# larq/compute-engine

Hardware: AMD Instinct MI355X
Metric: binary-MACs/sec (LceBconv2d 3x3 256->256, 56x56, batch 256/GPU, f32 out) (higher is better)
Workload: dtype fp4-e2m1 (exact +-1) matrix-core dot product, fp32 accumulate, f32 epilogue

## Files before the change

compute-engine_amd/csrc/lce_dispatch_stream.h:

```cpp
#pragma once
#include "../../include/lce_hip.h"
#include "lce_kernel_types.h"
#include "lce_kernels_stream.h"

namespace lce {

template <int DST, bool FAST, bool CLAMP, bool SIGN, bool I8F>
stream_fn stream_by_kch(int kch, bool strips) {
  if (strips)
    return kch == 4 ? bconv2d_stream<DST, 3, 3, 4, FAST, CLAMP, SIGN, false, true, I8F> : nullptr;
  switch (kch) {
    case 8: return bconv2d_stream<DST, 3, 3, 8, FAST, CLAMP, SIGN, true, false, I8F>;
    case 4: return bconv2d_stream<DST, 3, 3, 4, FAST, CLAMP, SIGN, false, false, I8F>;
    case 2: return bconv2d_stream<DST, 3, 3, 2, FAST, CLAMP, SIGN, false, false, I8F>;
    case 1: return bconv2d_stream<DST, 3, 3, 1, FAST, CLAMP, SIGN, false, false, I8F>;
    default: return nullptr;
  }
}
template <int DST, bool CLAMP, bool SIGN, bool I8F = false>
stream_fn stream_by_fast(int kch, bool fast, bool strips) {
  return fast ? stream_by_kch<DST, true, CLAMP, SIGN, I8F>(kch, strips) : stream_by_kch<DST, false, CLAMP, SIGN, I8F>(kch, strips);
}
template <int DST, bool CLAMP, bool I8F>
stream_fn find_stream_part(int kch, bool fast, bool sign, bool strips) {
  if constexpr (DST == kDstBitpacked) return stream_by_fast<kDstBitpacked, false, false>(kch, fast, strips);
  else return sign ? stream_by_fast<DST, CLAMP, true, I8F>(kch, fast, strips) : stream_by_fast<DST, CLAMP, false, I8F>(kch, fast, strips);
}

}
```

compute-engine_amd/csrc/lce_kernel_args.h:

```cpp
#pragma once
#include <stdint.h>
#include "lce_experiments.h"

namespace lce {

enum : int { kDstFloat = 0, kDstInt8 = 1, kDstBitpacked = 2 };

enum : int {
  kZeroPadNone = 0,
  kZeroPadExact = 1,
  kZeroPadCorrection = 2,
};

struct FastDiv {
  uint32_t magic;
  uint32_t shift;
};

inline FastDiv make_fastdiv(uint32_t d) {
  FastDiv f{0u, 0u};
  if (d <= 1) return f;
  uint32_t l = 0;
  while ((1ull << l) < d) ++l;
  const uint64_t two = 1ull << (31 + l);
  f.magic = (uint32_t)((two + d - 1) / d);
  f.shift = l - 1;
  return f;
}
struct FastDivNB {
  uint32_t magic;
  uint32_t shift;
  uint32_t pass;
};
inline FastDivNB make_fastdiv_nb(uint32_t d) {
  const FastDiv f = make_fastdiv(d);
  return FastDivNB{f.magic, f.shift, f.magic == 0u ? 0xffffffffu : 0u};
}

struct ConvArgs {
  int32_t H, W;
  int32_t Cw, Cwg;
  int32_t OH, OW;
  int32_t N, Npg;
  int32_t KH, KW, SH, SW, DH, DW, PH, PW;
  int32_t M;
  int32_t PT, NT;
  int32_t Wout;
  uint32_t in_bytes;
  FastDiv div_ow, div_oh;
  int32_t clamp_min, clamp_max;
  int32_t zero_pad_mode;
  int32_t bzp;
  int32_t eKH, eKW;
  int32_t left_off, top_off;
};


struct MfmaArgs {
  int32_t H, W, Cw, Cin;
  int32_t Hp, Wp, PH, PW;
  uint32_t NPIX;
  int32_t CPW;
  int32_t KCH;
  int32_t Npad;
  int32_t zero_border;
  uint32_t x_bytes, w_bytes;
  FastDiv div_npix, div_wp, div_hp;
  float a_bt;
  float cmin, cmax;
  int32_t TPI;
  int32_t OHOW;
  int32_t halo_rows;
  int32_t PS;
  int32_t halo_bytes;
  int32_t QG;
  int32_t IPT;
  int32_t B;
  int32_t HPIX;
  int32_t f32_wide;
  int32_t i8_wide;
  int32_t noclamp;
  float bit_thr;
  FastDiv div_tpi, div_qg, div_ohow, div_hpix;
  FastDiv div_npg;
  int32_t Wh, TX;
  FastDiv div_wh, div_tx;
};


struct PwArgs {
  int32_t M;
  int32_t N;
  int32_t Npad;
  int32_t Cw;
  int32_t Cin;
  int32_t Wout;
  int32_t tiles;
  int32_t noclamp;
  uint32_t in_bytes;
  uint32_t out_bytes;
  float a_bt;
  float cmin, cmax;
  float bit_thr;
  int32_t OW, OHW;
  int32_t IW, IHW;
  int32_t SH, SW;
  FastDiv div_ow, div_ohw;
};



constexpr int kStreamItemsPerLane = 2;
struct StreamArgs {
  int32_t H, W, Cw, Cin;
  int32_t OH, OW, N, Npad, Wout;
  int32_t SH, SW, PH, PW;
  int32_t B;
  int32_t Wp;
  int32_t pitch;
  int32_t R;
  int32_t ring_bytes;
  int32_t zero_border;
  int32_t QG;
  int32_t IPR;
  int32_t RS;
  int32_t SPI;
  int32_t SRS;
  int32_t PBS;
  int32_t S;
  int32_t SPB;
  int32_t GSTR, G0M, GX;
  int32_t pph_log;
  int32_t NSTRIP, RSEG, WSo, XS0;
  int32_t flat;
  int32_t NPX;
  int32_t NQ;
  uint32_t need0;
  uint32_t in_bytes, w_bytes, out_bytes;
  uint32_t tab_bytes, tab_lim, tab_ctx, tab_sgn;
  uint32_t tab_seg;
  uint32_t sign_bytes;
  float a_bt, cmin, cmax, bit_thr;
  FastDivNB div_ipr, div_qg, div_srs, div_spi, div_r, div_rseg, div_gstr;
};


struct WsArgs {
  int32_t H, W, Cw, Cin;
  int32_t OH, OW, N, Npad, Wout;
  int32_t SH, SW, PH, PW;
  int32_t B;
  int32_t IPB;
  int32_t GROUPS;
  int32_t PARTS;
  int32_t NPXG;
  int32_t NQ;
  int32_t Hp, Wp;
  int32_t pitch, img_pitch;
  int32_t QG;
  int32_t items;
  int32_t zero_border;
  int32_t noclamp;
  uint32_t lds_images;
  uint32_t in_bytes, w_bytes, out_bytes, sign_bytes, tab_bytes;
  uint32_t tab_part, tab_ctx;
  float a_bt, cmin, cmax, bit_thr;
  FastDivNB div_qg, div_wp, div_hp, div_groups;
};

}
```

compute-engine_amd/csrc/lce_kernel_types.h:

```cpp
#pragma once
#include <stdint.h>
#include "../../include/lce_hip.h"
#include "lce_kernel_args.h"

namespace lce {

typedef void (*tiled_fn)(const ConvArgs, const uint32_t*, const uint32_t*, const float*,
                         const float*, const int32_t*, const int32_t*, const float*, void*);
typedef void (*general_fn)(const ConvArgs, const uint32_t*, const uint32_t*, const float*,
                           const float*, const int32_t*, const float*, void*);
typedef void (*mfma_fn)(const ConvArgs, const MfmaArgs, const uint8_t*, const uint8_t*, const float*,
                        const float*, const float*, const float*, void*, uint32_t*);
typedef void (*pointwise_fn)(const PwArgs, const uint32_t*, const uint8_t*, const float*, const float*, const float*, void*, uint32_t*);
typedef void (*stream_fn)(const StreamArgs, const uint8_t*, const uint8_t*, const float*, const float*, const float*,
                          const uint32_t*, void*, uint32_t*);

typedef void (*wstream_fn)(const WsArgs, const uint8_t*, const uint8_t*, const float*, const float*, const float*,
                           const uint32_t*, void*, uint32_t*);

tiled_fn lookup_tiled(int dst, int tm, int tn, int ch);
general_fn lookup_general(int dst);
mfma_fn lookup_mfma_workspace(int dst, int bm, int bn, bool zero_pad_correction);
mfma_fn lookup_mfma_direct(int dst, int bm, int bn, bool zero_pad_correction);
mfma_fn lookup_mfma_direct_2d(int dst, int bm, int bn, bool zero_pad_correction);
inline mfma_fn lookup_mfma(int dst, int bm, int bn, bool zero_pad_correction, bool direct, bool tile2d) {
  if (direct && tile2d) return lookup_mfma_direct_2d(dst, bm, bn, zero_pad_correction);
  return direct ? lookup_mfma_direct(dst, bm, bn, zero_pad_correction) : lookup_mfma_workspace(dst, bm, bn, zero_pad_correction);
}
int launch_expand_fp4(unsigned grid_x, void* stream, const uint32_t* in, void* workspace, const MfmaArgs& G, uint64_t chunks);
pointwise_fn lookup_pointwise(int dst, int nc, int nj, bool strided, bool i8_floor);
stream_fn lookup_stream_f32(int kch, bool fast, bool sign, bool strips);
stream_fn lookup_stream_f32_clamp(int kch, bool fast, bool sign, bool strips);
stream_fn lookup_stream_i8(int kch, bool fast, bool sign, bool strips);
stream_fn lookup_stream_i8_floor(int kch, bool fast, bool sign, bool strips);
stream_fn lookup_stream_bitpacked(int kch, bool fast, bool strips);
inline stream_fn lookup_stream(int dst, int kch, bool fast, bool clamp, bool sign, bool strips, bool i8_floor) {
  switch (dst) {
    case LCE_HIP_F32: return clamp ? lookup_stream_f32_clamp(kch, fast, sign, strips) : lookup_stream_f32(kch, fast, sign, strips);
    case LCE_HIP_I8: return i8_floor ? lookup_stream_i8_floor(kch, fast, sign, strips) : lookup_stream_i8(kch, fast, sign, strips);
    default: return lookup_stream_bitpacked(kch, fast, strips);
  }
}
wstream_fn lookup_wstream_f32(int kch, int nb, bool sign);
wstream_fn lookup_wstream_i8(int kch, int nb, bool sign);
wstream_fn lookup_wstream_i8_floor(int kch, int nb, bool sign);
wstream_fn lookup_wstream_bitpacked(int kch, int nb);
inline wstream_fn lookup_wstream(int dst, int kch, int nb, bool sign, bool i8_floor) {
  switch (dst) {
    case LCE_HIP_F32: return lookup_wstream_f32(kch, nb, sign);
    case LCE_HIP_I8: return i8_floor ? lookup_wstream_i8_floor(kch, nb, sign) : lookup_wstream_i8(kch, nb, sign);
    default: return lookup_wstream_bitpacked(kch, nb);
  }
}
int mfma_selftest_wstream();
int mfma_selftest_pointwise();
int mfma_selftest_stream();

inline bool stream_fast(const StreamArgs& G) {
  return (G.Cin == 64 || G.Cin == 128 || G.Cin == 256 || G.Cin == 512) && !G.zero_border;
}
inline bool stream_clamps(const StreamArgs& G) { return !(G.cmin <= 0.0f && G.cmax >= 2.0f * G.a_bt); }

}
```

compute-engine_amd/csrc/lce_kernels_stream.h:

```cpp
#pragma once
#include <lce_device_intrinsics.h>
#include "lce_kernel_args.h"
#include "lce_kernels.h"
#include "lce_kernels_mfma.h"
#include "lce_stream_stamps.h"

namespace lce {

template <int DD>
LCE_DEVICE uint32_t fp4_full_dword(uint32_t word) {
  constexpr uint32_t sel = DD == 0 ? 0x04000400u : DD == 1 ? 0x05010501u : DD == 2 ? 0x06020602u : 0x07030703u;
  const uint32_t u = pk_lshr_b16<0, 4>(perm_b32(word >> 2, word, sel)) & 0x03030303u;
  return perm_b32(0u, 0xAAA22A22u, u);
}

constexpr int stream_unit_lo(int units, int i, int n) { return units * i / n; }

constexpr int stream_blocks_per_cu(int dst, int kch, bool ksplit, bool strips) {
  return dst == kDstBitpacked && kch == 1 && !ksplit && !strips ? 2 : 1;
}
template <int DST, int KH, int KW, int KCH, bool FAST, bool CLAMP, bool SIGN, bool KSPLIT = false, bool STRIPS = false, bool I8F = false>
LCE_KERNEL void __launch_bounds__(256, stream_blocks_per_cu(DST, KCH, KSPLIT, STRIPS))
bconv2d_stream(const StreamArgs G, const uint8_t* __restrict__ xin, const uint8_t* __restrict__ wq,
               const float* __restrict__ mul, const float* __restrict__ bias, const float* __restrict__ thrf,
               const uint32_t* __restrict__ tabs, void* __restrict__ out, uint32_t* __restrict__ sign_words) {
  static_assert(!SIGN || DST != kDstBitpacked, "a bitpacked-output plan already writes bits");
  constexpr int KCHW = KSPLIT ? KCH / 2 : KCH;
  constexpr bool FLATC = KSPLIT;
  constexpr int KS = KH * KW * KCHW;
  constexpr int PS = KCH * 32 + 16;
  static_assert(!KSPLIT || KCH % 2 == 0, "the K split halves the chunks of a tap");
  constexpr int GA = 4;
  constexpr int NG = (KS + GA - 1) / GA;
  static_assert(KH == 3, "the context table holds three tap-row addresses");
  static_assert(KS >= 8 && KS * 8 <= 288, "the filter bank must fit the register file");

  const int tid = thread_idx_x();
  const int lane = tid & (kWave - 1), wave = uniform(tid >> 6);
  const int l31 = lane & 31, half = lane >> 5;
  const int nslb = KSPLIT ? 2 : 4 >> G.pph_log;
  const int slice = wave & (nslb - 1), pp = KSPLIT ? 0 : wave >> (2 - G.pph_log);
  const int khalf = KSPLIT ? wave >> 1 : 0;
  const int n0 = (block_idx_y() * nslb + slice) * 64;
  const bool slice_ok = n0 < G.Npad;
  const int nown = n0 + khalf * 32;

  uint8_t* const lds0 = lds_base();
  constexpr int SCW = KSPLIT ? 32 : 64;
  constexpr int SCRB = DST == kDstBitpacked && !KSPLIT ? 0 : 32 * SCW * 4;
  float* const scratch = (float*)(lds0 + G.ring_bytes) + wave * (32 * SCW);
  constexpr uint32_t kDumpStride = DST == kDstBitpacked && KCH == 1 ? 32u : 64u;
  const uint32_t dump = (uint32_t)G.ring_bytes + 4u * (uint32_t)SCRB + (uint32_t)lane * kDumpStride;
  uint8_t* const inbox = lds0 + G.ring_bytes + 4 * SCRB + 4096 + wave * 8192;
  uint8_t* const outbox = lds0 + G.ring_bytes + 4 * SCRB + 4096 + (wave ^ 2) * 8192;

  LCE_SPH(0);
  const int g0 = block_idx_x() * G.G0M;
  int nseg = G.S - g0;
  nseg = nseg <= 0 ? 0 : (int)fastdiv_nb((uint32_t)(nseg + G.GSTR - 1), G.div_gstr);
  nseg = nseg > G.SPB ? G.SPB : nseg;
  const int nblk_all = FLATC && G.flat ? (nseg * G.NPX + 31) >> 5 : nseg * G.PBS;
  const int nblk = slice_ok ? nblk_all : 0;
  const int usteps = (nblk_all + (1 << G.pph_log) - 1) >> G.pph_log;
  int dyn_last = FLATC && G.flat && ((nseg * G.NPX) & 31) != 0 ? nblk_all - 1 : -1;
  int dyn_lim = nseg * G.NPX - (nblk_all - 1) * 32 - 1;
  keep_in_vgpr(dyn_last);
  keep_in_vgpr(dyn_lim);
  const int ntile = (usteps + 3) >> 2;
  const uint32_t* const sched = tabs;
  const rsrc_t rtab = make_rsrc(tabs, G.tab_bytes);

  const rsrc_t rin = make_rsrc(xin, G.in_bytes);
  struct Issue {
    uint32_t s, rem, x, gl, g, img, slot, t, strip;
    int c0, iy, ix, cseg;
    bool on, inside;
  };
  constexpr int kIssueChunks = 12;
  auto issue_chunk = [&](auto cc_, Issue& I, uint32_t e, uint32_t e_end, u32x4& wv, uint32_t& dst, int& meta) LCE_LAMBDA_INLINE {
    constexpr int c = decltype(cc_)::value;
    if constexpr (c == 0) {
      I.on = e < e_end;
      I.s = fastdiv_nb(e, G.div_ipr);
    } else if constexpr (c == 1) {
      I.rem = e - I.s * (uint32_t)G.IPR;
      I.x = fastdiv_nb(I.rem, G.div_qg);
    } else if constexpr (c == 2) {
      I.c0 = (int)(I.rem - I.x * (uint32_t)G.QG) * 4;
      I.gl = fastdiv_nb(I.s, G.div_srs);
    } else if constexpr (c == 3) {
      I.g = (uint32_t)g0 + I.gl * (uint32_t)G.GSTR;
      I.img = fastdiv_nb(I.g, G.div_spi);
    } else if constexpr (c == 4) {
      I.cseg = (int)(I.g - I.img * (uint32_t)G.SPI);
      I.iy = (int)(I.s - I.gl * (uint32_t)G.SRS) - G.PH;
      if constexpr (STRIPS) I.strip = fastdiv_nb((uint32_t)I.cseg, G.div_rseg);
    } else if constexpr (c == 5) {
      if constexpr (STRIPS) {
        I.cseg -= (int)I.strip * G.RSEG;
        I.ix = (int)I.x + (int)I.strip * (G.WSo * G.SW) - G.XS0;
        I.iy += I.cseg * (G.RS * G.SH);
        I.inside = I.on && (uint32_t)I.iy < (uint32_t)G.H && (uint32_t)I.ix < (uint32_t)G.W && I.img < (uint32_t)G.B;
      } else {
        I.iy += I.cseg * (G.RS * G.SH);
        I.inside = I.on && (uint32_t)I.iy < (uint32_t)G.H && I.img < (uint32_t)G.B;
      }
    } else if constexpr (c == 6) {
      I.slot = I.s - fastdiv_nb(I.s, G.div_r) * (uint32_t)G.R;
    } else if constexpr (c == 7) {
      I.t = I.slot * (uint32_t)G.pitch + ((uint32_t)G.PW + I.x) * (uint32_t)PS;
    } else if constexpr (c == 8) {
      dst = I.on ? I.t + (uint32_t)I.c0 * 16u : dump;
      meta = I.c0 | (I.inside ? 0x100 : 0);
    } else if constexpr (c == 9) {
      I.t = (uint32_t)((int)I.img * G.H + I.iy) * (uint32_t)G.W;
    } else if constexpr (c == 10) {
      I.t = (I.t + (STRIPS ? (uint32_t)I.ix : I.x)) * (uint32_t)G.Cw * 4u + (uint32_t)I.c0 * 4u;
    } else {
      const uint32_t off = I.t;
      if constexpr (FAST && KCH == 1) {
        const u32x2 v2 = buf_load(rin, I.inside ? off : kOobOffset, (u32x2*)nullptr);
        wv[0] = v2[0]; wv[1] = v2[1]; wv[2] = 0u; wv[3] = 0u;
      } else if (FAST || (G.Cw & 3) == 0) {
        wv = buf_load(rin, I.inside ? off : kOobOffset, (u32x4*)nullptr);
      } else {
#pragma unroll
        for (int q = 0; q < 4; ++q) wv[q] = buf_load(rin, I.inside && I.c0 + q < G.Cw ? off + 4u * q : kOobOffset, (uint32_t*)nullptr);
      }
    }
  };
  auto item_issue = [&](uint32_t e, uint32_t e_end, u32x4& wv, uint32_t& dst, int& meta) LCE_LAMBDA_INLINE {
    Issue I;
    issue_chunk(IntC<0>{}, I, e, e_end, wv, dst, meta); issue_chunk(IntC<1>{}, I, e, e_end, wv, dst, meta);
    issue_chunk(IntC<2>{}, I, e, e_end, wv, dst, meta); issue_chunk(IntC<3>{}, I, e, e_end, wv, dst, meta);
    issue_chunk(IntC<4>{}, I, e, e_end, wv, dst, meta); issue_chunk(IntC<5>{}, I, e, e_end, wv, dst, meta);
    issue_chunk(IntC<6>{}, I, e, e_end, wv, dst, meta); issue_chunk(IntC<7>{}, I, e, e_end, wv, dst, meta);
    issue_chunk(IntC<8>{}, I, e, e_end, wv, dst, meta); issue_chunk(IntC<9>{}, I, e, e_end, wv, dst, meta);
    issue_chunk(IntC<10>{}, I, e, e_end, wv, dst, meta); issue_chunk(IntC<11>{}, I, e, e_end, wv, dst, meta);
    static_assert(kIssueChunks == 12, "calls above");
  };
  auto item_write_word = [&](auto qc, const u32x4& wv, uint32_t dst, int meta) LCE_LAMBDA_INLINE {
    constexpr int q = decltype(qc)::value;
    if constexpr (q < (KCH * 2 < 4 ? KCH * 2 : 4)) {
      u32x4 v;
      if constexpr (FAST) {
        v = fp4_of_full_word(wv[q]);
      } else {
        const int cc = (meta & 0xff) + q;
        int valid = G.Cin - cc * 32;
        valid = valid < 0 ? 0 : (valid > 32 ? 32 : valid);
        if (!(meta & 0x100) && G.zero_border) valid = 0;
        v = valid == 32 ? fp4_of_full_word(wv[q]) : fp4_of_word(wv[q], valid);
        if (cc >= KCH * 2) return;
      }
      *(u32x4*)(lds0 + dst + q * 16) = v;
    }
  };
  auto item_write = [&](const u32x4& wv, uint32_t dst, int meta) LCE_LAMBDA_INLINE {
    item_write_word(IntC<0>{}, wv, dst, meta);
    item_write_word(IntC<1>{}, wv, dst, meta);
    item_write_word(IntC<2>{}, wv, dst, meta);
    item_write_word(IntC<3>{}, wv, dst, meta);
  };
  u32x4 pv = {0u, 0u, 0u, 0u};
  auto write_chunk = [&](auto cc_, const u32x4& wv, uint32_t dst, int meta) LCE_LAMBDA_INLINE {
    constexpr int c = decltype(cc_)::value, q = c >> 2, dd = c & 3;
    if constexpr (q < (KCH * 2 < 4 ? KCH * 2 : 4)) {
      if constexpr (FAST) {
        pv[dd] = fp4_full_dword<dd>(wv[q]);
        if constexpr (dd == 3) *(u32x4*)(lds0 + dst + q * 16) = pv;
      } else {
        if constexpr (dd == 3) item_write_word(IntC<q>{}, wv, dst, meta);
      }
    }
  };

  u32x4 W[KS][2];
  const rsrc_t rw = make_rsrc(wq, G.w_bytes);
  auto bank_loads = [&](auto ac, auto bc) LCE_LAMBDA_INLINE {
    constexpr int a = decltype(ac)::value, b = decltype(bc)::value;
#pragma unroll
    for (int i = a; i < b; ++i)
    {
      const int ksl = i >> 1, ksg = KSPLIT ? (ksl / KCHW) * KCH + khalf * KCHW + ksl % KCHW : ksl;
      const int jt = KSPLIT ? (i & 1) ^ khalf : (i & 1);
#ifdef LCE_ST_NOBANK
      W[i >> 1][i & 1] = buf_load(rw, slice_ok && ksg < 0 ? (uint32_t)jt : kOobOffset, (u32x4*)nullptr);
#else
      W[i >> 1][i & 1] = buf_load(rw, slice_ok ? (uint32_t)((ksg * 2 + half) * G.Npad + n0 + jt * 32 + l31) * 16u : kOobOffset, (u32x4*)nullptr);
#endif
    }
    sched_fence();
  };
  constexpr bool kBankPaced = KSPLIT;
  constexpr int kBankAhead = 12;
  constexpr int kBankFirst = kBankPaced ? 2 * kBankAhead : KS / 2;
  constexpr int kBankRest = kBankPaced ? 0 : 2 * KS - kBankFirst;
  static_assert(kBankFirst <= 2 * KS, "the first run is part of the bank");
  auto bank_run = [&](auto rc) LCE_LAMBDA_INLINE { bank_loads(IntC<0>{}, IntC<kBankFirst>{}); };
  auto bank_piece = [&](auto pc) LCE_LAMBDA_INLINE {
    constexpr int p = decltype(pc)::value;
    if constexpr (!kBankPaced) bank_loads(IntC<kBankFirst + kBankRest * p / 16>{}, IntC<kBankFirst + kBankRest * (p + 1) / 16>{});
  };
  sched_fence();
  if constexpr (!kBankPaced) bank_run(IntC<0>{});
  const uint32_t need0 = kBankPaced ? G.need0 : sched[0];
  u32x4 wv0[4];
  uint32_t dv0[4];
  int mv0[4];
#pragma unroll
  for (int k = 0; k < 4; ++k) item_issue((uint32_t)(k * 256 + tid), need0, wv0[k], dv0[k], mv0[k]);
  if constexpr (kBankPaced) bank_run(IntC<0>{});
  LCE_SPH(58);

  LCE_SPH(59);
  float tj[2], uj[2];
  f32x2 mj[2], bj[2];
#pragma unroll
  for (int j = 0; j < 2; ++j) {
    const int n = slice_ok ? n0 + (KSPLIT ? j ^ khalf : j) * 32 + l31 : 0;
    tj[j] = uj[j] = 0.0f;
    mj[j] = f32x2{0.0f, 0.0f};
    bj[j] = f32x2{0.0f, 0.0f};
    if constexpr (DST == kDstBitpacked) tj[j] = thrf[n];
    else { mj[j] = f32x2{mul[n], mul[n]}; bj[j] = f32x2{bias[n], bias[n]}; }
    if constexpr (DST == kDstInt8) { tj[j] = thrf[n]; uj[j] = thrf[G.Npad + n]; }
  }
  f32x16 kbt = f32x16_fill(khalf ? 0.0f : G.a_bt);
  pin(kbt);
  float cminv = G.cmin, cmaxv = G.cmax;
  keep_in_vgpr(cminv);
  keep_in_vgpr(cmaxv);

  if constexpr (!STRIPS) {
    const uint32_t code = G.zero_border ? 0u : 0x22222222u;
    const u32x4 v = {code, code, code, code};
    const int padc = G.Wp - G.W;
    constexpr int CH = KCH * 2;
    for (int e = tid; e < G.R * padc * CH; e += 256) {
      const int c16 = e % CH, t = e / CH, pc = t % padc, slot = t / padc;
      const int px = pc < G.PW ? pc : pc + G.W;
      *(u32x4*)(lds0 + (size_t)slot * G.pitch + (size_t)px * PS + c16 * 16) = v;
    }
  }
  block_barrier_keep_vm();
  LCE_SPH(60);
  sched_fence();
  auto item_write_with_bank = [&](auto kc, const u32x4& wv, uint32_t dst, int meta) LCE_LAMBDA_INLINE {
    constexpr int k = decltype(kc)::value;
    item_write_word(IntC<0>{}, wv, dst, meta);
    sched_fence();
    bank_piece(IntC<4 * k + 0>{});
    item_write_word(IntC<1>{}, wv, dst, meta);
    sched_fence();
    bank_piece(IntC<4 * k + 1>{});
    item_write_word(IntC<2>{}, wv, dst, meta);
    sched_fence();
    bank_piece(IntC<4 * k + 2>{});
    item_write_word(IntC<3>{}, wv, dst, meta);
    sched_fence();
    bank_piece(IntC<4 * k + 3>{});
  };
  item_write_with_bank(IntC<0>{}, wv0[0], dv0[0], mv0[0]);
  item_write_with_bank(IntC<1>{}, wv0[1], dv0[1], mv0[1]);
  item_write_with_bank(IntC<2>{}, wv0[2], dv0[2], mv0[2]);
  item_write_with_bank(IntC<3>{}, wv0[3], dv0[3], mv0[3]);
  for (uint32_t e0 = 4u * 256u; e0 < need0; e0 += 4u * 256u) {
#pragma unroll
    for (int k = 0; k < 4; ++k) item_issue(e0 + (uint32_t)(k * 256 + tid), need0, wv0[k], dv0[k], mv0[k]);
#pragma unroll
    for (int k = 0; k < 4; ++k) item_write(wv0[k], dv0[k], mv0[k]);
  }
  LCE_SPH(61);
  constexpr uint32_t kItemB = KSPLIT ? 512u : 256u;
  u32x4 pwa, pwb = {0u, 0u, 0u, 0u}, pwc = {0u, 0u, 0u, 0u};
  uint32_t pda, pdb = dump, pdc = dump;
  int pma, pmb = 0, pmc = 0;
  bool have_b;
  {
    const uint32_t a = sched[0], b = sched[1];
    item_issue(a + (uint32_t)tid, b, pwa, pda, pma);
    if constexpr (KSPLIT) item_issue(a + (uint32_t)(256 + tid), b, pwc, pdc, pmc);
    have_b = b - a > kItemB;
    if (have_b) item_issue(a + kItemB + (uint32_t)tid, b, pwb, pdb, pmb);
  }
  auto bank_home = [&](auto ksc) LCE_LAMBDA_INLINE {
    constexpr int ks = decltype(ksc)::value;
#pragma unroll
    for (int j = 0; j < 2; ++j) {
      if (ks < 32 && stream_blocks_per_cu(DST, KCH, KSPLIT, STRIPS) == 1) keep_in_agpr(W[ks][j]);
      else keep_in_vgpr(W[ks][j]);
    }
  };
  block_barrier_keep_vm();
  LCE_SPH(1);

  struct Ctx {
    u32x4 t;
    uint32_t s;
    uint32_t m;
    uint32_t bo, bs;
  };
  const uint32_t row_bytes = DST == kDstBitpacked ? (uint32_t)G.Wout * 4u : (uint32_t)G.N * (DST == kDstInt8 ? 1u : 4u);
  const rsrc_t rout = make_rsrc(out, G.out_bytes);
  constexpr int LPR = DST == kDstFloat ? (KSPLIT ? 8 : 16) : DST == kDstInt8 ? (KSPLIT ? 2 : 4) : 64;
  constexpr int RPI = 64 / LPR;
  uint32_t chan_off;
  if constexpr (DST == kDstFloat) {
    const int n = (KSPLIT ? nown : n0) + (lane & (LPR - 1)) * 4;
    chan_off = n < G.N ? (uint32_t)n * 4u : kOobOffset;
  } else if constexpr (DST == kDstInt8) {
    const int n = (KSPLIT ? nown : n0) + (lane & (LPR - 1)) * 16;
    chan_off = n < G.N ? (uint32_t)n : kOobOffset;
  } else if constexpr (KSPLIT) {
    chan_off = lane < 32 && (nown >> 5) < G.Wout ? (uint32_t)(nown >> 5) * 4u : kOobOffset;
  } else {
    chan_off = lane < 32 ? (uint32_t)(n0 >> 5) * 4u : kOobOffset;
  }
  const uint32_t first_px = STRIPS ? 0u : (uint32_t)g0 * (uint32_t)(G.RS * G.OW);
  uint32_t* const segbase = (uint32_t*)(lds0 + G.ring_bytes + 4 * SCRB + 4096);
  if constexpr (STRIPS) {
    for (int gl = tid; gl < G.SPB; gl += 256) {
      const uint32_t g = (uint32_t)(g0 + gl * G.GSTR);
      const uint32_t img = fastdiv_nb(g, G.div_spi), rem = g - img * (uint32_t)G.SPI;
      const uint32_t strip = fastdiv_nb(rem, G.div_rseg), rowseg = rem - strip * (uint32_t)G.RSEG;
      const uint32_t px = (img * (uint32_t)G.OH + rowseg * (uint32_t)G.RS) * (uint32_t)G.OW + strip * (uint32_t)G.WSo;
      segbase[2 * gl + 0] = px * row_bytes;
      segbase[2 * gl + 1] = px * (uint32_t)G.Wout * 4u;
    }
    block_barrier_keep_vm();
  }
  chan_off += first_px * row_bytes;
  const int nq = G.NQ;
  auto load_ctx = [&](int u, Ctx& cx) LCE_LAMBDA_INLINE {
    int q = (u << G.pph_log) + pp;
    q = q < nq ? q : nq - 1;
    cx.t = buf_load(rtab, (uint32_t)G.tab_ctx + (uint32_t)(q * 64 + lane) * 16u, (u32x4*)nullptr);
    if constexpr (SIGN) cx.s = buf_load(rtab, (uint32_t)G.tab_sgn + (uint32_t)(q * 64 + lane) * 4u, (uint32_t*)nullptr);
    else cx.s = 0u;
    cx.m = FLATC && (u << G.pph_log) + pp == dyn_last ? 0x80000000u : 0u;
    cx.bo = cx.bs = 0u;
    if constexpr (STRIPS) {
      const int gl = (int)tabs[G.tab_seg / 4 + q];
      cx.bo = segbase[2 * gl + 0];
      if constexpr (SIGN) cx.bs = segbase[2 * gl + 1];
    }
  };
  const rsrc_t rsgn = make_rsrc(sign_words, SIGN ? G.sign_bytes : 0u);
  const uint32_t sign_chan_off = lane < 32 && (!KSPLIT || (nown >> 5) < G.Wout)
                                     ? (uint32_t)((KSPLIT ? nown : n0) >> 5) * 4u + first_px * (uint32_t)G.Wout * 4u
                                     : kOobOffset;
  auto sign_base = [&](int u, const Ctx& cx) LCE_LAMBDA_INLINE -> uint32_t {
    const int q = (u << G.pph_log) + pp;
    return sat_add_u32((cx.s | cx.m) + cx.bs, q < nblk ? sign_chan_off : kOobOffset);
  };
  float bit_thrv[2];
#pragma unroll
  for (int j = 0; j < 2; ++j) bit_thrv[j] = n0 + (KSPLIT ? j ^ khalf : j) * 32 + l31 < G.N ? G.bit_thr : -__builtin_inff();
  auto out_base = [&](int u, const Ctx& cx) LCE_LAMBDA_INLINE -> uint32_t {
    const int q = (u << G.pph_log) + pp;
    return sat_add_u32((cx.t[3] | cx.m) + cx.bo, q < nblk ? chan_off : kOobOffset);
  };

  auto transform2 = [&](f32x2 x, f32x2 m, f32x2 b) LCE_LAMBDA_INLINE -> f32x2 {
#ifdef LCE_STREAM_PK_F32
    return mul_then_add_pk(x, m, b);
#else
    f32x2 y = {mul_then_add(x[0], m[0], b[0]), mul_then_add(x[1], m[1], b[1])};
    return y;
#endif
  };
  f32x4 yb[8];
  u32x4 pk[2];
  uint32_t bw[2] = {0u, 0u};
  constexpr int NUA = (KSPLIT && DST != kDstBitpacked) ? 8 : 16;
  constexpr bool kTight = SIGN && !FAST && KCH >= 4;
  constexpr bool kPipeBallots = KSPLIT || KS * 4 / 9 >= 16 || DST != kDstFloat;
  unsigned long long pend[2] = {0ull, 0ull};
  auto flush_ballots = [&](auto Tc) LCE_LAMBDA_INLINE {
    constexpr int T = decltype(Tc)::value;
    if constexpr (DST == kDstBitpacked) {
      constexpr int q = (T & 3) + 8 * (T >> 2);
#pragma unroll
      for (int j = 0; j < (KSPLIT ? 1 : 2); ++j) {
        bw[j] = write_lane_settled<q>((uint32_t)pend[j], bw[j]);
        bw[j] = write_lane_settled<q + 4>((uint32_t)(pend[j] >> 32), bw[j]);
      }
    } else {
      constexpr int j = KSPLIT ? 0 : T >> 3, r0 = (T & 7) * 2, q0 = (r0 & 3) + 8 * (r0 >> 2);
      bw[j] = write_lane_settled<q0>((uint32_t)pend[0], bw[j]);
      bw[j] = write_lane_settled<q0 + 4>((uint32_t)(pend[0] >> 32), bw[j]);
      bw[j] = write_lane_settled<q0 + 1>((uint32_t)pend[1], bw[j]);
      bw[j] = write_lane_settled<q0 + 5>((uint32_t)(pend[1] >> 32), bw[j]);
    }
  };
  auto epi_a = [&](auto tc, f32x16 (&acc)[2], auto pipe_) LCE_LAMBDA_INLINE {
    constexpr int t = decltype(tc)::value;
    constexpr bool PIPE = decltype(pipe_)::value != 0 && kPipeBallots;
    if constexpr (DST == kDstBitpacked && KSPLIT) {
      constexpr int r = t, q = (r & 3) + 8 * (r >> 2);
      unsigned long long bits[1];
      bits[0] = wave_ballot(acc[0][r] > tj[0]);
      if constexpr (PIPE) {
        if constexpr (t > 0) { hold_until(pend[0], bits[0], bits[0]); flush_ballots(IntC<(t > 0 ? t - 1 : 0)>{}); }
        pend[0] = bits[0];
      } else {
        settle_ballots(bits);
        bw[0] = write_lane_settled<q>((uint32_t)bits[0], bw[0]);
        bw[0] = write_lane_settled<q + 4>((uint32_t)(bits[0] >> 32), bw[0]);
      }
    } else if constexpr (DST == kDstBitpacked) {
      constexpr int r = t, q = (r & 3) + 8 * (r >> 2);
      unsigned long long bits[2];
#pragma unroll
      for (int j = 0; j < 2; ++j) bits[j] = wave_ballot(acc[j][r] > tj[j]);
      if constexpr (PIPE) {
        if constexpr (t > 0) {
          hold_until(pend[0], bits[0], bits[1]);
          hold_until(pend[1], bits[0], bits[1]);
          flush_ballots(IntC<(t > 0 ? t - 1 : 0)>{});
        }
        pend[0] = bits[0];
        pend[1] = bits[1];
      } else {
        settle_ballots(bits);
#pragma unroll
        for (int j = 0; j < 2; ++j) {
          bw[j] = write_lane_settled<q>((uint32_t)bits[j], bw[j]);
          bw[j] = write_lane_settled<q + 4>((uint32_t)(bits[j] >> 32), bw[j]);
        }
      }
    } else {
      constexpr int j = KSPLIT ? 0 : t >> 3, r0 = (t & 7) * 2;
      const int row0 = (r0 & 3) + 8 * (r0 >> 2) + 4 * half;
      f32x2 y;
      if constexpr (DST == kDstFloat) {
        f32x2 x = {acc[j][r0], acc[j][r0 + 1]};
        if constexpr (CLAMP) { x[0] = med3(x[0], cminv, cmaxv); x[1] = med3(x[1], cminv, cmaxv); }
        y = transform2(x, mj[j], bj[j]);
      } else {
        const f32x2 x = {acc[j][r0], acc[j][r0 + 1]};
        if constexpr (I8F) { y[0] = fma1(x[0], mj[j][0], bj[j][0]); y[1] = fma1(x[1], mj[j][1], bj[j][1]); }
        else y = transform2(x, mj[j], bj[j]);
        y[0] = med3(y[0], tj[j], uj[j]);
        y[1] = med3(y[1], tj[j], uj[j]);
      }
      scratch[row0 * SCW + j * 32 + l31] = y[0];
      scratch[(row0 + 1) * SCW + j * 32 + l31] = y[1];
      if constexpr (SIGN) {
        unsigned long long bits[2];
        bits[0] = wave_ballot(y[0] < bit_thrv[j]);
        bits[1] = wave_ballot(y[1] < bit_thrv[j]);
        if constexpr (PIPE) {
          if constexpr (t > 0) {
            hold_until(pend[0], bits[0], bits[1]);
            hold_until(pend[1], y[0], y[1]);
            flush_ballots(IntC<(t > 0 ? t - 1 : 0)>{});
          }
          pend[0] = bits[0];
          pend[1] = bits[1];
        } else {
          settle_ballots(bits);
          constexpr int q0 = (r0 & 3) + 8 * (r0 >> 2);
          bw[j] = write_lane_settled<q0>((uint32_t)bits[0], bw[j]);
          bw[j] = write_lane_settled<q0 + 4>((uint32_t)(bits[0] >> 32), bw[j]);
          bw[j] = write_lane_settled<q0 + 1>((uint32_t)bits[1], bw[j]);
          bw[j] = write_lane_settled<q0 + 5>((uint32_t)(bits[1] >> 32), bw[j]);
        }
      }
    }
  };
  auto sign_store = [&](uint32_t sob) LCE_LAMBDA_INLINE {
    if constexpr (KSPLIT) {
      buf_store1(rsgn, sob, bw[0]);
    } else if ((G.Wout & 1) == 0) {
      const u32x2 v = {bw[0], bw[1]};
      buf_store2(rsgn, sob, v);
    } else {
      buf_store1(rsgn, sob, bw[0]);
      buf_store1(rsgn, (n0 >> 5) + 1 < G.Wout ? sat_add_u32(sob, 4u) : kOobOffset, bw[1]);
    }
  };
  auto epi_b_read = [&](auto kc) LCE_LAMBDA_INLINE {
    constexpr int k = decltype(kc)::value;
    if constexpr (DST == kDstFloat) {
      yb[k] = *(const f32x4*)(scratch + ((lane / LPR) + RPI * k) * SCW + (lane & (LPR - 1)) * 4);
    } else if constexpr (DST == kDstInt8) {
      yb[k] = *(const f32x4*)(scratch + ((lane / LPR) + RPI * (k >> 2)) * SCW + (lane & (LPR - 1)) * 16 + (k & 3) * 4);
    }
  };
  auto epi_b = [&](auto kc) LCE_LAMBDA_INLINE {
    if constexpr (!kTight) epi_b_read(kc);
  };
  auto epi_c = [&](auto kc, uint32_t ob) LCE_LAMBDA_INLINE {
    constexpr int k = decltype(kc)::value;
    if constexpr (kTight) epi_b_read(kc);
    if constexpr (DST == kDstFloat) {
      buf_store_streaming_so(rout, ob, (uint32_t)(RPI * k) * row_bytes, yb[k]);
    } else if constexpr (DST == kDstInt8) {
#pragma unroll
      for (int i = 0; i < 4; ++i) if constexpr (!I8F) yb[k][i] = yb[k][i] + __builtin_copysignf(0x1.fffffep-2f, yb[k][i]);
      if constexpr ((k & 1) == 1) {
        uint32_t lo, hi;
        if constexpr (I8F) cvt_rpi_pack8_i8(yb[k - 1], yb[k], lo, hi);
        else cvt_pack8_i8(yb[k - 1], yb[k], lo, hi);
        pk[k >> 2][(k & 3) - 1] = lo;
        pk[k >> 2][k & 3] = hi;
      }
      if constexpr ((k & 3) == 3) buf_store_so(rout, ob, (uint32_t)(RPI * (k >> 2)) * row_bytes, pk[k >> 2]);
    } else {
      if constexpr (k == 0) {
        if constexpr (KSPLIT) {
          buf_store1(rout, ob, bw[0]);
        } else if ((G.Wout & 1) == 0) {
          const u32x2 v = {bw[0], bw[1]};
          buf_store2(rout, ob, v);
        } else {
          buf_store1(rout, ob, bw[0]);
          buf_store1(rout, (n0 >> 5) + 1 < G.Wout ? sat_add_u32(ob, 4u) : kOobOffset, bw[1]);
        }
      }
    }
  };
  auto epi_partial = [&](int u, const Ctx& cx) LCE_LAMBDA_INLINE {
    int q = (u << G.pph_log) + pp;
    if (q >= nblk) return;
    const uint32_t lim1 = q == dyn_last ? (uint32_t)dyn_lim : tabs[G.tab_lim / 4 + q];
    const uint32_t base = (cx.t[3] & 0x7fffffffu) + chan_off;
    if constexpr (DST == kDstFloat) {
      const uint32_t rowl = (uint32_t)(lane / LPR);
#pragma unroll
      for (int k = 0; k < 32 / RPI; ++k) {
        const uint32_t row = rowl + (uint32_t)(RPI * k);
        buf_store_streaming(rout, row <= lim1 ? base + (row - rowl) * row_bytes : kOobOffset, yb[k]);
      }
    } else if constexpr (DST == kDstInt8) {
      const uint32_t rowl = (uint32_t)(lane / LPR);
#pragma unroll
      for (int k = 0; k < 32 / RPI; ++k) {
        const uint32_t row = rowl + (uint32_t)(RPI * k);
        buf_store(rout, row <= lim1 ? base + (row - rowl) * row_bytes : kOobOffset, pk[k]);
      }
    } else {
      const uint32_t rowl = (uint32_t)(lane & 31);
      const uint32_t o = rowl <= lim1 ? base : kOobOffset;
      buf_store1(rout, o, bw[0]);
      if constexpr (!KSPLIT) buf_store1(rout, (n0 >> 5) + 1 < G.Wout ? sat_add_u32(o, 4u) : kOobOffset, bw[1]);
    }
    if constexpr (SIGN) {
      const uint32_t rowl = (uint32_t)(lane & 31);
      sign_store(rowl <= lim1 ? sat_add_u32(cx.s & 0x7fffffffu, sign_chan_off) : kOobOffset);
    }
  };
  constexpr int XS = KSPLIT ? 10 : 0;
  constexpr int NUB = KSPLIT ? 4 : 8;
  constexpr int SA0 = XS, SA = SA0 + (KSPLIT ? NUA : KS * 4 / 9);
  constexpr int SB0 = (SA + GA - 1) / GA * GA, SBN = KSPLIT ? 4 : (KS * 2 + 8) / 9, SC0 = KS - SBN;
  static_assert(SA < KS - 1, "phase layout");
  constexpr int SBG_avail = (SC0 - SB0) / GA * 2 + ((SC0 - SB0) % GA > 2 ? (SC0 - SB0) % GA - 2 : 0);
  constexpr int SBG = SBG_avail >= 4 ? 4 : (SBG_avail >= 2 ? 2 : 1);
  static_assert(SA <= SB0 && SB0 <= SC0 && (SBG_avail >= 1 || DST == kDstBitpacked), "phase layout");

  f32x4 xch[4];
  auto x_send = [&](auto qc, f32x16 (&set)[2], int slot) LCE_LAMBDA_INLINE {
    constexpr int q = decltype(qc)::value;
    const f32x4 v = {set[1][4 * q], set[1][4 * q + 1], set[1][4 * q + 2], set[1][4 * q + 3]};
    *(f32x4*)(outbox + slot * 4096 + q * 1024 + lane * 16) = v;
  };
  auto x_recv = [&](int slot) LCE_LAMBDA_INLINE {
#pragma unroll
    for (int q = 0; q < 4; ++q) xch[q] = *(const f32x4*)(inbox + slot * 4096 + q * 1024 + lane * 16);
  };
  auto x_add = [&](auto qc, f32x16 (&set)[2]) LCE_LAMBDA_INLINE {
    constexpr int q = decltype(qc)::value;
#pragma unroll
    for (int i = 0; i < 4; ++i) set[0][4 * q + i] += xch[q][i];
  };

  f32x16 acc[2][2];
#pragma unroll
  for (int a = 0; a < 2; ++a)
#pragma unroll
    for (int j = 0; j < 2; ++j) acc[a][j] = kbt;

  Ctx cur, nxt;
  load_ctx(0, cur);
  uint32_t epi_ob = kOobOffset;
  bool epi_part = false;
  int epi_u = 0;
  Ctx epi_cx = cur;
  u32x4 af[2][GA];

  auto ctx_khalf = [&](Ctx& cx) LCE_LAMBDA_INLINE {
    if constexpr (KSPLIT) {
      const uint32_t koff = (uint32_t)khalf * (uint32_t)(KCHW * 32);
      cx.t[0] += koff; cx.t[1] += koff; cx.t[2] += koff;
    }
  };
  ctx_khalf(cur);
  auto frag_addr = [&](const Ctx& cx, int ks) LCE_LAMBDA_INLINE -> uint32_t {
    const int fy = ks / (KW * KCHW), fx = (ks / KCHW) % KW, kc = ks % KCHW;
    return cx.t[fy] + (uint32_t)(fx * PS + kc * 32);
  };

  constexpr int NPG = KS - SA - 1;
  uint32_t next_ob = kOobOffset, next_sob = kOobOffset, epi_sob = kOobOffset;
  bool next_part = false;
  Issue isa, isc;
  auto step = [&](auto kc_, auto first_, int u, uint32_t sch1, uint32_t sch2) LCE_LAMBDA_INLINE {
    constexpr int k = decltype(kc_)::value, PAR = k & 1;
    constexpr bool FIRST = decltype(first_)::value != 0;
    static_assert(!FIRST || k == 0, "the first block step is step 0 of tile step 0");
    if constexpr (k == 0) {
#pragma unroll
      for (int d = GA - 1; d >= 0; --d) af[0][d] = *(const u32x4*)(lds0 + frag_addr(cur, d));
    }
    auto kstep = [&](auto ksc) LCE_LAMBDA_INLINE {
      constexpr int ks = decltype(ksc)::value;
      if constexpr (ks < KS) {
        constexpr int g = ks / GA;
        constexpr int fs = (g + k * NG) & 1;
        if constexpr (FIRST) bank_home(IntC<ks>{});
        if constexpr (ks == 0) acc[PAR][0] = mfma_fp4_32x32x64_unscaled(af[fs][0], W[0][0], kbt);
        else acc[PAR][0] = mfma_fp4_32x32x64_unscaled(af[fs][ks % GA], W[ks][0], acc[PAR][0]);
        pin(acc[PAR][0]);
        sched_fence();
#ifndef LCE_ST_NOFRAG
        if constexpr (ks % GA < 2) {
          constexpr int d1 = GA - 1 - 2 * (ks % GA), d0 = d1 - 1;
          if constexpr (g + 1 < NG) {
            if constexpr ((g + 1) * GA + d1 < KS) af[fs ^ 1][d1] = *(const u32x4*)(lds0 + frag_addr(cur, (g + 1) * GA + d1));
            if constexpr ((g + 1) * GA + d0 < KS) af[fs ^ 1][d0] = *(const u32x4*)(lds0 + frag_addr(cur, (g + 1) * GA + d0));
          } else if constexpr (k < 3) {
            af[fs ^ 1][d1] = *(const u32x4*)(lds0 + frag_addr(nxt, d1));
            af[fs ^ 1][d0] = *(const u32x4*)(lds0 + frag_addr(nxt, d0));
            if constexpr (KS - (NG - 1) * GA < 2) {
              af[fs ^ 1][1] = *(const u32x4*)(lds0 + frag_addr(nxt, 1));
              af[fs ^ 1][0] = *(const u32x4*)(lds0 + frag_addr(nxt, 0));
            }
          }
        }
#endif
#ifndef LCE_ST_NOEPI
        if constexpr (!FIRST && ks >= SB0 && ks % GA >= 2 && (ks - SB0) / GA * 2 + (ks % GA - 2) < SBG) {
          constexpr int slot = (ks - SB0) / GA * 2 + (ks % GA - 2);
          constexpr int lo = stream_unit_lo(NUB, slot, SBG), hi = stream_unit_lo(NUB, slot + 1, SBG);
          if constexpr (slot == 0) wave_lds_scratch_fence();
#ifndef LCE_ST_NOEPI_B
          if constexpr (lo + 0 < hi) epi_b(IntC<lo + 0>{});
          if constexpr (lo + 1 < hi) epi_b(IntC<lo + 1>{});
          if constexpr (lo + 2 < hi) epi_b(IntC<lo + 2>{});
          if constexpr (lo + 3 < hi) epi_b(IntC<lo + 3>{});
          if constexpr (lo + 4 < hi) epi_b(IntC<lo + 4>{});
          if constexpr (lo + 5 < hi) epi_b(IntC<lo + 5>{});
          if constexpr (lo + 6 < hi) epi_b(IntC<lo + 6>{});
          if constexpr (lo + 7 < hi) epi_b(IntC<lo + 7>{});
#endif
        }
#endif
        if constexpr (ks == 1) {
          next_ob = out_base(u, cur);
          if constexpr (SIGN) next_sob = sign_base(u, cur);
          next_part = (int)(uniform(cur.t[3] | cur.m) >> 31) != 0;
        }
        sched_fence();
        if constexpr (ks == 0) acc[PAR][1] = mfma_fp4_32x32x64_unscaled(af[fs][0], W[0][1], kbt);
        else acc[PAR][1] = mfma_fp4_32x32x64_unscaled(af[fs][ks % GA], W[ks][1], acc[PAR][1]);
        pin(acc[PAR][1]);
        sched_fence();
#ifndef LCE_ST_NOEPI
        if constexpr (KSPLIT && !FIRST && ks < XS) {
          constexpr int slot = (k + 1) & 1;
          if constexpr (ks < 4) x_send(IntC<ks>{}, acc[PAR ^ 1], slot);
          else if constexpr (ks == 4) block_barrier_keep_vm();
          else if constexpr (ks == 5) x_recv(slot);
          else x_add(IntC<ks - 6>{}, acc[PAR ^ 1]);
        }
        if constexpr (!FIRST && ks >= SA0 && ks < SA) {
          constexpr int lo = stream_unit_lo(NUA, ks - SA0, SA - SA0), hi = stream_unit_lo(NUA, ks - SA0 + 1, SA - SA0);
          if constexpr (lo == 0) wave_lds_order();
#ifndef LCE_ST_NOEPI_A
          if constexpr (lo + 0 < hi) epi_a(IntC<lo + 0>{}, acc[PAR ^ 1], IntC<1>{});
          if constexpr (lo + 1 < hi) epi_a(IntC<lo + 1>{}, acc[PAR ^ 1], IntC<1>{});
          if constexpr (lo + 2 < hi) epi_a(IntC<lo + 2>{}, acc[PAR ^ 1], IntC<1>{});
          if constexpr (lo + 3 < hi) epi_a(IntC<lo + 3>{}, acc[PAR ^ 1], IntC<1>{});
#endif
          static_assert(hi - lo <= 4, "units per gap");
        }
        if constexpr (!FIRST && ks >= SC0) {
          constexpr int lo = stream_unit_lo(NUB, ks - SC0, SBN), hi = stream_unit_lo(NUB, ks - SC0 + 1, SBN);
#ifndef LCE_ST_NOEPI_C
          if constexpr (lo + 0 < hi) epi_c(IntC<lo + 0>{}, epi_ob);
          if constexpr (lo + 1 < hi) epi_c(IntC<lo + 1>{}, epi_ob);
          if constexpr (lo + 2 < hi) epi_c(IntC<lo + 2>{}, epi_ob);
          if constexpr (lo + 3 < hi) epi_c(IntC<lo + 3>{}, epi_ob);
#endif
        }
#endif
        if constexpr (kBankPaced && FIRST && ks + kBankAhead < KS) bank_loads(IntC<2 * (ks + kBankAhead)>{}, IntC<2 * (ks + kBankAhead) + 2>{});
        if constexpr (kPipeBallots && (SIGN || DST == kDstBitpacked) && !FIRST && ks == SA) flush_ballots(IntC<NUA - 1>{});
        if constexpr (SIGN && !FIRST && ks == SA) sign_store(epi_sob);
        if constexpr (ks == SA) load_ctx(u + 1, nxt);
        if constexpr (KSPLIT && ks == (NG - 1) * GA - 1) ctx_khalf(nxt);
#ifndef LCE_ST_NOPROD
        if constexpr (ks > SA) {
          if constexpr (k == 0) {
            constexpr int lo = stream_unit_lo(16, ks - SA - 1, NPG), hi = stream_unit_lo(16, ks - SA, NPG);
            if constexpr (lo + 0 < hi) write_chunk(IntC<lo + 0>{}, pwa, pda, pma);
            if constexpr (lo + 1 < hi) write_chunk(IntC<lo + 1>{}, pwa, pda, pma);
            if constexpr (lo + 2 < hi) write_chunk(IntC<lo + 2>{}, pwa, pda, pma);
            if constexpr (lo + 3 < hi) write_chunk(IntC<lo + 3>{}, pwa, pda, pma);
            static_assert(hi - lo <= 4, "chunks per gap");
          } else if constexpr (k == 1) {
            constexpr int lo = stream_unit_lo(kIssueChunks, ks - SA - 1, NPG), hi = stream_unit_lo(kIssueChunks, ks - SA, NPG);
            if constexpr (lo + 0 < hi) issue_chunk(IntC<lo + 0>{}, isa, sch1 + (uint32_t)tid, sch2, pwa, pda, pma);
            if constexpr (lo + 1 < hi) issue_chunk(IntC<lo + 1>{}, isa, sch1 + (uint32_t)tid, sch2, pwa, pda, pma);
            if constexpr (lo + 2 < hi) issue_chunk(IntC<lo + 2>{}, isa, sch1 + (uint32_t)tid, sch2, pwa, pda, pma);
            static_assert(hi - lo <= 3, "chunks per gap");
          } else if constexpr (KSPLIT && k == 2) {
            constexpr int lo = stream_unit_lo(16, ks - SA - 1, NPG), hi = stream_unit_lo(16, ks - SA, NPG);
            if constexpr (lo + 0 < hi) write_chunk(IntC<lo + 0>{}, pwc, pdc, pmc);
            if constexpr (lo + 1 < hi) write_chunk(IntC<lo + 1>{}, pwc, pdc, pmc);
            if constexpr (lo + 2 < hi) write_chunk(IntC<lo + 2>{}, pwc, pdc, pmc);
            if constexpr (lo + 3 < hi) write_chunk(IntC<lo + 3>{}, pwc, pdc, pmc);
          } else if constexpr (KSPLIT && k == 3) {
            constexpr int lo = stream_unit_lo(kIssueChunks, ks - SA - 1, NPG), hi = stream_unit_lo(kIssueChunks, ks - SA, NPG);
            if constexpr (lo + 0 < hi) issue_chunk(IntC<lo + 0>{}, isc, sch1 + (uint32_t)(256 + tid), sch2, pwc, pdc, pmc);
            if constexpr (lo + 1 < hi) issue_chunk(IntC<lo + 1>{}, isc, sch1 + (uint32_t)(256 + tid), sch2, pwc, pdc, pmc);
            if constexpr (lo + 2 < hi) issue_chunk(IntC<lo + 2>{}, isc, sch1 + (uint32_t)(256 + tid), sch2, pwc, pdc, pmc);
          }
        }
#endif
        sched_fence();
      }
    };
    kstep(IntC<0>{}); kstep(IntC<1>{}); kstep(IntC<2>{}); kstep(IntC<3>{}); kstep(IntC<4>{}); kstep(IntC<5>{});
    kstep(IntC<6>{}); kstep(IntC<7>{}); kstep(IntC<8>{}); kstep(IntC<9>{}); kstep(IntC<10>{}); kstep(IntC<11>{});
    kstep(IntC<12>{}); kstep(IntC<13>{}); kstep(IntC<14>{}); kstep(IntC<15>{}); kstep(IntC<16>{}); kstep(IntC<17>{});
    kstep(IntC<18>{}); kstep(IntC<19>{}); kstep(IntC<20>{}); kstep(IntC<21>{}); kstep(IntC<22>{}); kstep(IntC<23>{});
    kstep(IntC<24>{}); kstep(IntC<25>{}); kstep(IntC<26>{}); kstep(IntC<27>{}); kstep(IntC<28>{}); kstep(IntC<29>{});
    kstep(IntC<30>{}); kstep(IntC<31>{}); kstep(IntC<32>{}); kstep(IntC<33>{}); kstep(IntC<34>{}); kstep(IntC<35>{});
    static_assert(KS <= 36, "kstep calls above");
    if constexpr (!FIRST) {
      if (epi_part) epi_partial(epi_u, epi_cx);
    }
    epi_ob = next_ob;
    epi_sob = next_sob;
    epi_part = next_part;
    epi_u = u;
    epi_cx = cur;
    cur = nxt;
  };

  using TagFirst = IntC<1>;
  using TagSteady = IntC<0>;
  auto tile_step = [&](auto first_, int T) LCE_LAMBDA_INLINE {
    const uint32_t sch1 = sched[T + 1], sch2 = sched[T + 2];
    step(IntC<0>{}, first_, 4 * T + 0, sch1, sch2);
    if (4 * T + 1 < usteps) step(IntC<1>{}, TagSteady{}, 4 * T + 1, sch1, sch2);
    if (4 * T + 2 < usteps) step(IntC<2>{}, TagSteady{}, 4 * T + 2, sch1, sch2);
    if (4 * T + 3 < usteps) step(IntC<3>{}, TagSteady{}, 4 * T + 3, sch1, sch2);
    if (have_b) item_write(pwb, pdb, pmb);
    have_b = sch2 - sch1 > kItemB;
    if (have_b) item_issue(sch1 + kItemB + (uint32_t)tid, sch2, pwb, pdb, pmb);
    block_barrier_keep_vm();
    LCE_SPH(2 + T);
  };
  if (ntile > 0) tile_step(TagFirst{}, 0);
  for (int T = 1; T < ntile; ++T) tile_step(TagSteady{}, T);

  auto drain = [&](f32x16 (&last)[2], int slot) LCE_LAMBDA_INLINE {
    if constexpr (KSPLIT) {
      x_send(IntC<0>{}, last, slot); x_send(IntC<1>{}, last, slot); x_send(IntC<2>{}, last, slot); x_send(IntC<3>{}, last, slot);
      block_barrier_keep_vm();
      x_recv(slot);
      x_add(IntC<0>{}, last); x_add(IntC<1>{}, last); x_add(IntC<2>{}, last); x_add(IntC<3>{}, last);
    }
    wave_lds_order();
    auto drain_a = [&](auto tc) LCE_LAMBDA_INLINE {
      if constexpr (decltype(tc)::value < NUA) epi_a(tc, last, IntC<0>{});
    };
    drain_a(IntC<0>{}); drain_a(IntC<1>{}); drain_a(IntC<2>{}); drain_a(IntC<3>{});
    drain_a(IntC<4>{}); drain_a(IntC<5>{}); drain_a(IntC<6>{}); drain_a(IntC<7>{});
    drain_a(IntC<8>{}); drain_a(IntC<9>{}); drain_a(IntC<10>{}); drain_a(IntC<11>{});
    drain_a(IntC<12>{}); drain_a(IntC<13>{}); drain_a(IntC<14>{}); drain_a(IntC<15>{});
    if constexpr (SIGN) sign_store(epi_sob);
    wave_lds_fence();
    auto drain_bc = [&](auto kc) LCE_LAMBDA_INLINE {
      if constexpr (decltype(kc)::value < NUB) epi_b(kc);
    };
    drain_bc(IntC<0>{}); drain_bc(IntC<1>{}); drain_bc(IntC<2>{}); drain_bc(IntC<3>{});
    drain_bc(IntC<4>{}); drain_bc(IntC<5>{}); drain_bc(IntC<6>{}); drain_bc(IntC<7>{});
    auto drain_c = [&](auto kc) LCE_LAMBDA_INLINE {
      if constexpr (decltype(kc)::value < NUB) epi_c(kc, epi_ob);
    };
    drain_c(IntC<0>{}); drain_c(IntC<1>{}); drain_c(IntC<2>{}); drain_c(IntC<3>{});
    drain_c(IntC<4>{}); drain_c(IntC<5>{}); drain_c(IntC<6>{}); drain_c(IntC<7>{});
    if (epi_part) epi_partial(epi_u, epi_cx);
  };
  if (usteps & 1) drain(acc[0], 0);
  else drain(acc[1], 1);
  LCE_SPH(63);
}

}
```

compute-engine_amd/csrc/lce_plan.cpp:

```cpp
#include "lce_plan.h"
#include "lce_plan_internal.h"
#include "lce_kernel_types.h"
#include <cstdio>
#include <cstdlib>

#include <limits.h>
#include <string.h>

#include <algorithm>
#include <cmath>
#include <initializer_list>
#include <limits>
#include <cstdio>

namespace lce {

static int out_size(int padding, int image, int filter, int stride, int dilation) {
  const int eff = (filter - 1) * dilation + 1;
  if (stride == 0) return 0;
  if (padding == LCE_HIP_PADDING_SAME) return (image + stride - 1) / stride;
  if (padding == LCE_HIP_PADDING_VALID) return (image + stride - eff) / stride;
  return 0;
}
static int pad_before(int stride, int dilation, int in, int filter, int out) {
  const int eff = (filter - 1) * dilation + 1;
  const int total = std::max(0, (out - 1) * stride + eff - in);
  return total / 2;
}

static void read_debug_environment(HostPlan& p) {
  const char* dbg = getenv("LCE_PLAN_DEBUG");
  p.dbg_level = dbg ? std::max(1, atoi(dbg)) : 0;
  p.dbg_no_wstream = getenv("LCE_PLAN_NO_WSTREAM") != nullptr;
  p.dbg_int8_exact = getenv("LCE_PLAN_INT8_EXACT") != nullptr;
  p.dbg_int8_full = getenv("LCE_PLAN_INT8_FULL") != nullptr;
  static bool table_printed = false;
  if (p.dbg_level >= 3 && !table_printed) { table_printed = true; dump_cost_table(stderr); }
}

std::string validate_and_infer(HostPlan& p) {
  const lce_hip_bconv2d_desc& d = p.d;
  char buf[256];
  read_debug_environment(p);
  if (d.batch < 0 || d.in_height < 1 || d.in_width < 1 || d.channels_in < 1 ||
      d.filter_height < 1 || d.filter_width < 1 || d.channels_out < 1)
    return "bconv2d: all tensor dimensions must be positive";
  if (d.stride_height < 1 || d.stride_width < 1 || d.dilation_height < 1 || d.dilation_width < 1)
    return "bconv2d: strides and dilations must be positive";
  if (d.padding != LCE_HIP_PADDING_SAME && d.padding != LCE_HIP_PADDING_VALID)
    return "bconv2d: padding must be SAME or VALID";
  if (d.pad_values != 0 && d.pad_values != 1)
    return "Attribute pad_values must be 0 or 1.";
  if (d.activation < LCE_HIP_ACT_NONE || d.activation > LCE_HIP_ACT_RELU6)
    return "bconv2d: unsupported fused activation";
  if (d.dst_type != LCE_HIP_F32 && d.dst_type != LCE_HIP_I8 && d.dst_type != LCE_HIP_BITPACKED)
    return "Supported output types are int8, int32, and float32.";
  if (d.groups < 1) return "bconv2d: groups must be >= 1";
  if (d.groups > 1) {
    if (d.channels_in % d.groups) return "bconv2d: channels_in must be divisible by groups";
    if ((d.channels_in / d.groups) % 32)
      return "bconv2d: group_size % core::bitpacking_bitwidth was not 0";
    if (d.channels_out % d.groups) return "bconv2d: channels_out % groups was not 0";
  }
  if (d.padding == LCE_HIP_PADDING_SAME && d.pad_values == 0) {
    const bool ok = (d.semantics == LCE_HIP_SEM_REFERENCE && d.channels_in % 2 == 0) ||
                    (d.semantics != LCE_HIP_SEM_REFERENCE && d.dst_type == LCE_HIP_F32 &&
                     d.activation == LCE_HIP_ACT_NONE);
    if (!ok)
      return "Zero-padding is only supported by the reference kernel with an even number of "
             "input channels, or when using float output with no fused activation function.";
  }
  if (d.dst_type == LCE_HIP_I8 && !(d.out_scale > 0.0f))
    return "bconv2d: int8 output needs a positive output scale";

  p.out_h = out_size(d.padding, d.in_height, d.filter_height, d.stride_height, d.dilation_height);
  p.out_w = out_size(d.padding, d.in_width, d.filter_width, d.stride_width, d.dilation_width);
  if (p.out_h < 1 || p.out_w < 1) {
    snprintf(buf, sizeof buf, "bconv2d: empty output (%d x %d)", p.out_h, p.out_w);
    return buf;
  }
  p.pad_h = pad_before(d.stride_height, d.dilation_height, d.in_height, d.filter_height, p.out_h);
  p.pad_w = pad_before(d.stride_width, d.dilation_width, d.in_width, d.filter_width, p.out_w);
  p.cw = ceil_div(d.channels_in, 32);
  p.cwg = ceil_div(d.channels_in / d.groups, 32);
  p.npg = d.channels_out / d.groups;
  p.wout = ceil_div(d.channels_out, 32);
  p.backtransform_add = d.filter_height * d.filter_width * (d.channels_in / d.groups);
  p.zero_pad_mode = kZeroPadNone;
  if (d.padding == LCE_HIP_PADDING_SAME && d.pad_values == 0)
    p.zero_pad_mode = d.semantics == LCE_HIP_SEM_REFERENCE ? kZeroPadExact : kZeroPadCorrection;
  const int64_t per_image_bytes = (int64_t)d.in_height * d.in_width * p.cw * 4;
  if (per_image_bytes >= (1ll << 31)) return "bconv2d: one input image must be smaller than 2 GiB";
  if ((int64_t)p.out_h * p.out_w >= (1ll << 31)) return "bconv2d: output plane too large";
  return "";
}

static int word_index(const char* s, std::initializer_list<const char*> words) {
  int i = 0;
  for (const char* w : words) {
    if (!strcmp(s, w)) return i;
    ++i;
  }
  return -1;
}

static bool int_value(const char* s, int* v) {
  *v = atoi(s);
  return *v != 0 || !strcmp(s, "0");
}

static bool in_set(int v, std::initializer_list<int> set) { return std::find(set.begin(), set.end(), v) != set.end(); }

std::string set_plan_option(HostPlan& p, const char* key, const char* value, unsigned* invalidates) {
  PlanOptions& o = p;
  const unsigned plan_and_upload = kStaleSelection | kStaleUpload;
  const unsigned all = plan_and_upload | kStalePacked | kStaleWeightImage;
  unsigned stale = 0;
  int v = 0;
  *invalidates = 0;
  if (!strcmp(key, "tile2d")) {
    if ((v = word_index(value, {"auto", "on", "off"})) < 0) return "plan_set_option: tile2d must be auto|on|off";
    o.tile2d_pref = v;
    stale = kStaleSelection;
  } else if (!strcmp(key, "pointwise_tiles")) {
    if (!int_value(value, &v) || v < 0 || v > 8) return "plan_set_option: pointwise_tiles must be 0 (auto) .. 8";
    o.pw_tiles_pref = v;
  } else if (!strcmp(key, "pointwise_channels")) {
    if (!int_value(value, &v) || !in_set(v, {0, 32, 64, 128}))
      return "plan_set_option: pointwise_channels must be 0 (auto), 32, 64 or 128";
    o.pw_nj_pref = v / 32;
    stale = kStaleSelection;
  } else if (!strcmp(key, "stream_rows")) {
    if (!int_value(value, &v) || v < 0) return "plan_set_option: stream_rows must be 0 (auto) or a positive row count";
    o.stream_rows_pref = v;
    stale = plan_and_upload;
  } else if (!strcmp(key, "stream_strip")) {
    if (!int_value(value, &v) || v < -1)
      return "plan_set_option: stream_strip must be -1 (auto), 0 (whole rows) or a strip width";
    o.stream_strip_pref = v;
    stale = plan_and_upload;
  } else if (!strcmp(key, "stream_interleave")) {
    if ((v = word_index(value, {"0", "1", "auto"})) < 0) return "plan_set_option: stream_interleave must be auto, 0 or 1";
    o.stream_interleave_pref = v == 2 ? -1 : v;
    stale = plan_and_upload;
  } else if (!strcmp(key, "stream_blocks_per_cu")) {
    if ((v = word_index(value, {"auto", "1", "2"})) < 0) return "plan_set_option: stream_blocks_per_cu must be auto, 1 or 2";
    o.stream_occ_pref = v;
    stale = plan_and_upload;
  } else if (!strcmp(key, "stream_flat")) {
    if ((v = word_index(value, {"0", "1"})) < 0) return "plan_set_option: stream_flat must be 0 or 1";
    o.stream_noflat = v == 0;
    stale = plan_and_upload;
  } else if (!strcmp(key, "stream_pixel_phases")) {
    if (!int_value(value, &v) || !in_set(v, {0, 1, 2, 4}))
      return "plan_set_option: stream_pixel_phases must be 0 (auto), 1, 2 or 4";
    o.stream_phases_pref = v;
    stale = plan_and_upload;
  } else if (!strcmp(key, "wstream_blocks") || !strcmp(key, "wstream_images")) {
    const bool blocks = key[8] == 'b';
    if (!int_value(value, &v) || v < 0 || (blocks && v > 4))
      return "plan_set_option: wstream_blocks must be 0 (auto) .. 4, wstream_images 0 (auto) or a positive count";
    (blocks ? o.ws_blocks_pref : o.ws_images_pref) = v;
    stale = plan_and_upload;
  } else if (!strcmp(key, "compute_units")) {
    if ((v = atoi(value)) < 1) return "plan_set_option: compute_units must be positive";
    p.num_cus = v;
    o.cus_forced = true;
    stale = plan_and_upload;
  } else if (!strcmp(key, "int8_rounding")) {
    if ((v = word_index(value, {"auto", "exact"})) < 0) return "plan_set_option: int8_rounding must be auto or exact";
    o.int8_exact_pref = v == 1;
    stale = plan_and_upload | kStaleWeightImage;
  } else if (!strcmp(key, "phase")) {
    if ((v = word_index(value, {"all", "expand", "gemm"})) < 0) return "plan_set_option: phase must be all|expand|gemm";
    o.phase = v;
  } else if (!strcmp(key, "epilogue")) {
    if ((v = word_index(value, {"auto", "tile", "wide"})) < 0) return "plan_set_option: epilogue must be auto|tile|wide";
    o.epilogue_pref = v;
  } else if (!strcmp(key, "engine")) {
    if ((v = word_index(value, {"auto", "valu", "mfma", "direct", "pointwise", "stream", "wstream"})) < 0)
      return "plan_set_option: engine must be auto|valu|mfma|direct|pointwise|stream|wstream";
    o.engine_pref = v;
    stale = all;
  } else if (!strcmp(key, "kernel")) {
    if ((v = word_index(value, {"auto", "tiled", "general"})) < 0) return "plan_set_option: kernel must be auto|tiled|general";
    o.kernel_pref = v;
    stale = all;
  } else if (!strcmp(key, "tile")) {
    int tm = 0, tn = 0;
    if (strcmp(value, "auto") && !(sscanf(value, "%dx%d", &tm, &tn) == 2 &&
                                   ((tn <= 32 && lookup_tiled(LCE_HIP_F32, tm, tn, 1)) || mfma_cfg_by_tile(tm, tn))))
      return "plan_set_option: tile must be auto, a xor-popcount tile (4x16|2x32|2x16|1x32|1x16) or, with engine=mfma, a block tile "
             "(256x256|256x128|512x64|128x256|128x128|256x64|128x64)";
    o.tile_pref = TileShape{tm, tn};
    stale = all;
  } else {
    return std::string("plan_set_option: unknown key '") + key + "'";
  }
  *invalidates = stale;
  return "";
}

static int popcount32(uint32_t x) { return __builtin_popcount(x); }

static void fill_zero_pad_cache(HostPlan& p, const float* post_mul) {
  const lce_hip_bconv2d_desc& d = p.d;
  const int ew = (d.filter_width - 1) * d.dilation_width + 1;
  const int eh = (d.filter_height - 1) * d.dilation_height + 1;
  const int cin_g = d.channels_in / d.groups;
  const int n = d.channels_out;
  p.zero_pad_cache.assign((size_t)4 * eh * ew * n, 0.0f);
  std::vector<float> tap_val((size_t)n * d.filter_height * d.filter_width);
  for (int oc = 0; oc < n; ++oc)
    for (int t = 0; t < d.filter_height * d.filter_width; ++t) {
      int pop = 0;
      const uint32_t* w = &p.filter[((size_t)oc * d.filter_height * d.filter_width + t) * p.cwg];
      for (int k = 0; k < p.cwg; ++k) pop += popcount32(w[k]);
      tap_val[(size_t)oc * d.filter_height * d.filter_width + t] = (float)(cin_g - 2 * pop);
    }
  for (int y = 0; y < eh; ++y)
    for (int x = 0; x < ew; ++x)
      for (int oc = 0; oc < n; ++oc) {
        float corr[4] = {0.f, 0.f, 0.f, 0.f};
        for (int fy = 0; fy < d.filter_height; ++fy)
          for (int fx = 0; fx < d.filter_width; ++fx) {
            const float cur = tap_val[((size_t)oc * d.filter_height + fy) * d.filter_width + fx];
            const int efx = d.dilation_width * fx, efy = d.dilation_height * fy;
            const bool top = efy < y, bot = (eh - efy) <= y;
            const bool left = efx < x, right = (ew - efx) <= x;
            if (top || left) corr[0] += cur;
            if (top || right) corr[1] += cur;
            if (bot || left) corr[2] += cur;
            if (bot || right) corr[3] += cur;
          }
        const float m = -1.0f * post_mul[oc];
        for (int k = 0; k < 4; ++k)
          p.zero_pad_cache[(((size_t)k * eh + y) * ew + x) * n + oc] = m * corr[k];
      }
}

static int round_sat_i8_host(float c) {
  c = c < -128.0f ? -128.0f : (c > 127.0f ? 127.0f : c);
  volatile float s = c + std::copysign(0x1.fffffep-2f, c);
  return (int)s;
}
float int8_below_threshold(int32_t zero_point) {
  if (zero_point <= -128) return -std::numeric_limits<float>::infinity();
  if (zero_point > 127) return std::numeric_limits<float>::infinity();
  auto from_key = [](int64_t k) {
    uint32_t u = k >= 0 ? (uint32_t)k : 0x80000000u | (uint32_t)(-k - 1);
    float f;
    memcpy(&f, &u, 4);
    return f;
  };
  auto to_key = [](float f) { uint32_t u; memcpy(&u, &f, 4); return (u & 0x80000000u) ? -(int64_t)(u & 0x7fffffffu) - 1 : (int64_t)u; };
  int64_t lo = to_key(-128.0f), hi = to_key(127.0f);
  while (hi - lo > 1) {
    const int64_t mid = lo + (hi - lo) / 2;
    if (round_sat_i8_host(from_key(mid)) >= zero_point) hi = mid; else lo = mid;
  }
  return from_key(hi);
}

void fold_parameters(HostPlan& p, const int32_t* filter_ohwi, const float* post_mul,
                     const float* post_bias, const int32_t* thresholds) {
  const lce_hip_bconv2d_desc& d = p.d;
  const int n = d.channels_out;
  const size_t fwords = (size_t)n * d.filter_height * d.filter_width * p.cwg;
  p.filter.assign((const uint32_t*)filter_ohwi, (const uint32_t*)filter_ohwi + fwords);
  p.mul.clear();
  p.bias.clear();
  p.thresholds.clear();
  p.zero_pad_cache.clear();
  if (d.dst_type == LCE_HIP_BITPACKED) {
    p.thresholds.assign(thresholds, thresholds + n);
  } else {
    const double scale = d.dst_type == LCE_HIP_I8 ? (double)d.out_scale : 1.0;
    const double zp = d.dst_type == LCE_HIP_I8 ? (double)d.out_zero_point : 0.0;
    const double a = (double)p.backtransform_add;
    p.mul.resize(n);
    p.bias.resize(n);
    for (int i = 0; i < n; ++i) {
      const double m = post_mul[i], b = post_bias[i];
      p.mul[i] = (float)(-1 * m / scale);
      p.bias[i] = (float)((b + a * m) / scale + zp);
    }
    int32_t lo = INT32_MIN, hi = INT32_MAX;
    switch (d.activation) {
      case LCE_HIP_ACT_RELU: lo = 0; break;
      case LCE_HIP_ACT_RELU6: lo = 0; hi = 6; break;
      case LCE_HIP_ACT_RELU_N1_TO_1: lo = -1; hi = 1; break;
      default: break;
    }
    lo = std::max(lo, -p.backtransform_add);
    hi = std::min(hi, p.backtransform_add);
    p.clamp_min = -hi + p.backtransform_add;
    p.clamp_max = -lo + p.backtransform_add;
    if (p.zero_pad_mode == kZeroPadCorrection) fill_zero_pad_cache(p, post_mul);
    p.bit_thr = d.dst_type == LCE_HIP_I8 ? int8_below_threshold(d.out_zero_point) : 0.0f;
  }
  p.have_weights = true;
  p.packed.clear();
  p.wq.clear();
}

bool tiled_supports(const HostPlan& p, int tn) {
  if (p.d.dst_type == LCE_HIP_BITPACKED && tn != 32) return false;
  if (p.d.groups > 1 && p.npg % tn != 0) return false;
  return true;
}

static void pack_for_tile(HostPlan& p) {
  const lce_hip_bconv2d_desc& d = p.d;
  const int tn = p.tile.tn, taps = d.filter_height * d.filter_width, n = d.channels_out;
  p.nt = ceil_div(n, tn);
  p.packed.assign((size_t)p.nt * taps * p.cwg * tn, 0u);
  p.oob_corr.assign((size_t)p.nt * taps * tn, 0);
  const int bzp = (d.channels_in / d.groups) / 2;
  for (int oc = 0; oc < n; ++oc) {
    const int t_idx = oc / tn, j = oc % tn;
    for (int t = 0; t < taps; ++t) {
      int pop = 0;
      for (int c = 0; c < p.cwg; ++c) {
        const uint32_t w = p.filter[((size_t)oc * taps + t) * p.cwg + c];
        p.packed[(((size_t)t_idx * taps + t) * p.cwg + c) * tn + j] = w;
        pop += popcount32(w);
      }
      p.oob_corr[((size_t)t_idx * taps + t) * tn + j] = bzp - pop;
    }
  }
  const size_t padded = (size_t)p.nt * tn;
  p.mul_p.assign(padded, 0.0f);
  p.bias_p.assign(padded, 0.0f);
  p.thr_p.assign(padded, INT32_MAX);
  std::copy(p.mul.begin(), p.mul.end(), p.mul_p.begin());
  std::copy(p.bias.begin(), p.bias.end(), p.bias_p.begin());
  std::copy(p.thresholds.begin(), p.thresholds.end(), p.thr_p.begin());
}

bool mfma_supported(const HostPlan& p) {
  const lce_hip_bconv2d_desc& d = p.d;
  if (d.groups != 1 && (d.channels_out / d.groups) % 64 != 0) return false;
  if (p.backtransform_add >= (1 << 23)) return false;
  const int cpad = ceil_div(d.channels_in, 64) * 64;
  const int64_t hp = padded_height(p), wp = padded_width(p);
  if (hp * wp * (cpad / 2) >= (1ll << 31)) return false;
  if (hp * wp * (cpad / 32) >= (1ll << 31)) return false;
  return true;
}

bool pointwise_supported(const HostPlan& p, int64_t pixels, int* nc, int* nj) {
  const lce_hip_bconv2d_desc& d = p.d;
  if (!mfma_supported(p)) return false;
  if (d.filter_height != 1 || d.filter_width != 1) return false;
  if (d.groups != 1 || p.pad_h != 0 || p.pad_w != 0) return false;
  if (p.out_h != (d.in_height - 1) / d.stride_height + 1 || p.out_w != (d.in_width - 1) / d.stride_width + 1) return false;
  if (d.channels_out % 32 != 0) return false;
  const int c = pointwise_bank_steps(ceil_div(d.channels_in, 64));
  if (c == 0) return false;
  const int t = d.channels_out / 32;
  int j = t % 4 == 0 ? 4 : t % 2 == 0 ? 2 : 1;
  if (c == 8 || d.dst_type == LCE_HIP_F32) j = std::min(j, 2);
  if (p.pw_nj_pref > 0) {
    if (t % p.pw_nj_pref != 0) return false;
    j = std::min(j, p.pw_nj_pref);
  } else {
    const int64_t tiles = (pixels + 31) / 32;
    if (j == 4 && tiles * (t / 4) < pw_small_launch_tiles) j = 2;
  }
  *nc = c;
  *nj = j;
  return true;
}

static bool pointwise_preferred(const HostPlan& p, int64_t pixels) {
  const int64_t tiles = (pixels + 31) / 32;
  if (p.d.dst_type == LCE_HIP_F32 && tiles * (p.d.channels_out / 64) >= 65536) return false;
  return pixels >= 1024;
}

PwArgs make_pw_args(const HostPlan& p, int batch_chunk) {
  const lce_hip_bconv2d_desc& d = p.d;
  PwArgs P{};
  const int64_t m = (int64_t)batch_chunk * p.out_h * p.out_w;
  P.M = (int32_t)m;
  P.N = d.channels_out;
  P.Npad = p.npad;
  P.Cw = p.cw;
  P.Cin = d.channels_in;
  P.Wout = p.wout;
  P.tiles = (int32_t)((m + 31) / 32);
  P.noclamp = (p.clamp_min <= 0 && (int64_t)p.clamp_max >= 2 * (int64_t)p.backtransform_add) ? 1 : 0;
  P.in_bytes = (uint32_t)((int64_t)batch_chunk * d.in_height * d.in_width * p.cw * 4);
  P.out_bytes = (uint32_t)std::min<int64_t>(out_bytes_of(p, batch_chunk), (1ll << 31) - 1);
  P.a_bt = (float)p.backtransform_add;
  P.cmin = (float)p.clamp_min;
  P.cmax = (float)p.clamp_max;
  P.bit_thr = p.bit_thr;
  P.OW = p.out_w;
  P.OHW = p.out_h * p.out_w;
  P.IW = d.in_width;
  P.IHW = d.in_height * d.in_width;
  P.SH = d.stride_height;
  P.SW = d.stride_width;
  P.div_ow = make_fastdiv((uint32_t)P.OW);
  P.div_ohw = make_fastdiv((uint32_t)P.OHW);
  return P;
}

static const MfmaCfg kMfmaCfgs[] = {
    {4, 2, 2, 4},
    {4, 2, 2, 2},
    {8, 1, 2, 2},
    {2, 2, 2, 4},
    {2, 2, 2, 2},
    {4, 1, 2, 2},
    {2, 1, 2, 2},
};
const MfmaCfg* mfma_cfg_by_tile(int bm, int bn) {
  for (const MfmaCfg& c : kMfmaCfgs)
    if (c.bm() == bm && c.bn() == bn) return &c;
  return nullptr;
}

int group_chunks(const lce_hip_bconv2d_desc& d) {
  const int cin_g = d.channels_in / d.groups;
  int most = 0;
  for (int g = 0; g < d.groups; ++g)
    most = std::max(most, ((g + 1) * cin_g + 63) / 64 - (g * cin_g) / 64);
  return most;
}

static void prepare_int8_epilogue(HostPlan& p) {
  const lce_hip_bconv2d_desc& d = p.d;
  const int n = d.channels_out, cin_g = d.channels_in / d.groups;
  p.mul_q.assign(p.npad, 0.0f);
  p.bias_q.assign(p.npad, 0.0f);
  std::copy(p.mul.begin(), p.mul.end(), p.mul_q.begin());
  std::copy(p.bias.begin(), p.bias.end(), p.bias_q.begin());
  for (int i = n; i < p.npad; ++i) p.bias_q[i] = std::numeric_limits<float>::infinity();
  p.thr_q.assign((size_t)2 * p.npad, 0.0f);
  const bool one_rounding = p.use_stream || p.use_wstream;
  auto two_roundings = [](float mul, float bias, int32_t x) {
    volatile float pr = (float)x * mul;
    volatile float r = pr + bias;
    return (float)r;
  };
  auto proven_form = [&](float mul, float bias, int32_t x) {
    return one_rounding ? std::fmaf((float)x, mul, bias) : two_roundings(mul, bias, x);
  };
  auto set_range = [&](int i, float mul, float bias, bool proven) {
    const float a0 = proven ? proven_form(mul, bias, p.clamp_min) : two_roundings(mul, bias, p.clamp_min);
    const float a1 = proven ? proven_form(mul, bias, p.clamp_max) : two_roundings(mul, bias, p.clamp_max);
    float lo = std::min(a0, a1), hi = std::max(a0, a1);
    if (!(lo == lo) || !(hi == hi)) { lo = -128.0f; hi = 127.0f; }
    p.thr_q[i] = std::max(-128.0f, std::min(127.0f, lo));
    p.thr_q[p.npad + i] = std::max(-128.0f, std::min(127.0f, hi));
  };
  for (int i = 0; i < n; ++i) set_range(i, p.mul[i], p.bias[i], false);
  p.int8_floor_ok = !p.int8_exact_pref && !p.dbg_int8_exact;
  p.int8_bias_adjusted = 0;
  const int32_t x_lo = std::max<int32_t>(0, p.clamp_min), x_hi = (int32_t)std::min<int64_t>(2 * (int64_t)p.backtransform_add, p.clamp_max);
  const bool even_only = cin_g % 2 == 0;
  auto sat8_half_away = [](float y) { const float r = std::round(y); return (int)std::max(-128.0f, std::min(127.0f, r)); };
  const int32_t first_even = even_only ? ((x_lo + 2) & ~1) : x_lo + 1;
  const int32_t n_mid = even_only ? (x_hi > first_even ? (x_hi - 1 - first_even) / 2 + 1 : 0) : std::max(0, x_hi - 1 - x_lo);
  const int32_t n_x = x_hi > x_lo ? n_mid + 2 : 1;
  auto x_at = [&](int32_t k) { return k == 0 ? x_lo : k == n_x - 1 ? x_hi : first_even + (even_only ? 2 : 1) * (k - 1); };
  auto inner_run = [&](auto&& y_of, float lo, float hi, int32_t* k0, int32_t* k1) {
    const bool inc = y_of(x_hi) >= y_of(x_lo);
    auto below = [&](int32_t k) { const float y = y_of(x_at(k)); return inc ? y <= lo : y >= hi; };
    auto not_past = [&](int32_t k) { const float y = y_of(x_at(k)); return inc ? y < hi : y > lo; };
    int32_t a = 0, b = n_x;
    while (a < b) { const int32_t m = a + (b - a) / 2; if (below(m)) a = m + 1; else b = m; }
    *k0 = a;
    b = n_x;
    while (a < b) { const int32_t m = a + (b - a) / 2; if (not_past(m)) a = m + 1; else b = m; }
    *k1 = a;
  };
  const bool check_all = p.dbg_int8_full;
  auto channel_ok = [&](int i, float mul, float bias, int32_t* bad_x) {
    const float a0 = proven_form(mul, bias, p.clamp_min), a1 = proven_form(mul, bias, p.clamp_max);
    if (!(a0 == a0) || !(a1 == a1)) return false;
    const float lo = std::max(-128.0f, std::min(127.0f, std::min(a0, a1))), hi = std::max(-128.0f, std::min(127.0f, std::max(a0, a1)));
    auto value_ok = [&](int32_t x) {
      float yc = proven_form(mul, bias, x);
      yc = yc < lo ? lo : (yc > hi ? hi : yc);
      const bool negative_tie = yc < 0.0f && yc - std::floor(yc) == 0.5f;
      if (!(yc == yc) || negative_tie ||
          (int)std::floor((double)yc + 0.5) != sat8_half_away(two_roundings(p.mul[i], p.bias[i], x))) {
        if (bad_x) *bad_x = x;
        return false;
      }
      return true;
    };
    int32_t k0, k1, r0, r1;
    inner_run([&](int32_t x) { return proven_form(mul, bias, x); }, lo, hi, &k0, &k1);
    inner_run([&](int32_t x) { return two_roundings(p.mul[i], p.bias[i], x); }, -128.5f, 127.5f, &r0, &r1);
    k0 = std::max(0, std::min(k0, r0) - 1);
    k1 = std::min(n_x, std::max(k1, r1) + 1);
    if (check_all) { k0 = 0; k1 = n_x; }
    if (!value_ok(x_lo) || !value_ok(x_hi)) return false;
    for (int32_t k = k0; k < k1; ++k)
      if (!value_ok(x_at(k))) return false;
    return true;
  };
  struct Adjusted { int i; float mul, bias; };
  std::vector<Adjusted> adjusted;
  for (int i = 0; i < n && p.int8_floor_ok; ++i) {
    int32_t bad = 0;
    if (channel_ok(i, p.mul[i], p.bias[i], &bad)) continue;
    const float y_bad = proven_form(p.mul[i], p.bias[i], bad), pr_bad = std::fabs((float)bad * p.mul[i]);
    const float big = std::max(std::max(pr_bad, std::fabs(p.bias[i])), std::fabs(y_bad));
    const float step = std::max(std::nextafter(big, INFINITY) - big, std::ldexp(1.0f, -20));
    bool found = false;
    for (int dm = 0; dm <= 4 && !found; ++dm) {
      float m2 = p.mul[i];
      for (int s = 0; s < (dm + 1) / 2; ++s) m2 = std::nextafter(m2, (dm & 1) ? INFINITY : -INFINITY);
      for (int t = 0; t < 9 && !found; ++t) {
        const int k = t < 5 ? t : 4 - t;
        if (dm == 0 && k == 0) continue;
        const float b2 = p.bias[i] - (float)k * step;
        if (channel_ok(i, m2, b2, nullptr)) { adjusted.push_back({i, m2, b2}); found = true; }
      }
    }
    if (!found) {
      if (p.dbg_level >= 1)
        fprintf(stderr,
                "[lce plan] int8: channel %d, accumulator %d -> y = %.9g: no neighbouring (multiplier, bias) reproduces the reference "
                "there, round-half-away instances\n",
                i, bad, (double)y_bad);
      p.int8_floor_ok = false;
    }
  }
  if (p.int8_floor_ok) {
    for (const auto& a : adjusted) { p.mul_q[a.i] = a.mul; p.bias_q[a.i] = a.bias; }
    for (int i = 0; i < n; ++i) set_range(i, p.mul_q[i], p.bias_q[i], true);
    p.int8_bias_adjusted = (int)adjusted.size();
    if (p.dbg_level >= 1 && !adjusted.empty())
      fprintf(stderr, "[lce plan] int8: one-instruction forms, %zu channel(s) with adjusted parameters\n", adjusted.size());
  }
}

static void pack_for_mfma(HostPlan& p) {
  const lce_hip_bconv2d_desc& d = p.d;
  const int taps = d.filter_height * d.filter_width, n = d.channels_out;
  const int bn = p.mfma.bn();
  const int cin_g = d.channels_in / d.groups;
  p.cpad = ((p.use_stream || p.use_wstream) ? stream_chunks(d) : ceil_div(d.channels_in, 64)) * 64;
  p.npad = ceil_div(n, bn) * bn;
  p.kch = d.groups > 1 ? group_chunks(d) : p.cpad / 64;
  const int kch = p.kch, ks_total = taps * kch;
  const int ks_alloc = (taps == 1 && d.groups == 1 && p.wq_layout == 0) ? pointwise_bank_steps(kch) : ks_total;
  p.wq.assign((size_t)std::max(ks_total, ks_alloc) * p.npad * 32, 0);
  for (int oc = 0; oc < n; ++oc) {
    const int g = oc / p.npg, chunk0 = (g * cin_g) / 64;
    for (int t = 0; t < taps; ++t)
      for (int ci = 0; ci < cin_g; ++ci) {
        const uint32_t w = p.filter[((size_t)oc * taps + t) * p.cwg + ci / 32];
        const uint8_t nib = ((w >> (ci % 32)) & 1u) ? 0x2 : 0xA;
        const int c = g * cin_g + ci;
        const int ks = t * kch + (c / 64 - chunk0), j = c % 64, half = j / 32, jj = j % 32;
        const size_t cell = p.wq_layout == 1 ? (((size_t)(oc / 32) * ks_total + ks) * 2 + half) * 32 + oc % 32
                                             : ((size_t)ks * 2 + half) * p.npad + oc;
        uint8_t& byte = p.wq[cell * 16 + jj / 2];
        byte |= (uint8_t)(nib << (4 * (jj & 1)));
      }
  }
  p.mul_q.assign(p.npad, 0.0f);
  p.bias_q.assign(p.npad, 0.0f);
  std::copy(p.mul.begin(), p.mul.end(), p.mul_q.begin());
  std::copy(p.bias.begin(), p.bias.end(), p.bias_q.begin());
  if (d.dst_type == LCE_HIP_I8) { prepare_int8_epilogue(p); return; }
  const int64_t a = p.backtransform_add;
  p.thr_q.assign(p.npad, (float)(2 * a + 2));
  for (size_t i = 0; i < p.thresholds.size(); ++i) {
    int64_t t = 2 * (int64_t)p.thresholds[i];
    t = std::max<int64_t>(-1, std::min<int64_t>(2 * a + 2, t));
    p.thr_q[i] = (float)t;
  }
}

MfmaCfg choose_mfma_cfg(const HostPlan& p, int64_t pixels) {
  const int n = p.d.channels_out;
  int bn = n > 128 ? 256 : n > 64 ? 128 : 64;
  auto blocks = [&](int bm, int bn_) { return ((pixels + bm - 1) / bm) * (int64_t)ceil_div(n, bn_); };
  while (bn > 64 && blocks(128, bn) < 512) bn /= 2;
  while (bn > 64 && p.d.groups > 1 && p.npg % bn) bn /= 2;
  const int bm = bn == 64 ? 256 : 128;
  const MfmaCfg* c = mfma_cfg_by_tile(bm, bn);
  if (bn == 64 && blocks(256, 64) < 512) c = mfma_cfg_by_tile(128, 64);
  return c ? *c : kMfmaCfgs[4];
}

bool direct_geometry(const HostPlan& p, const MfmaCfg& c, int* tpi, int* halo_rows, int* ps, int* halo_bytes,
                     int* ipt, int lds_budget, int* tile_tx, int* halo_w) {
  const lce_hip_bconv2d_desc& d = p.d;
  if (!mfma_supported(p)) return false;
  const int cpad = ceil_div(d.channels_in, 64) * 64;
  const int64_t wp = padded_width(p);
  const int bm = c.bm(), ohow = p.out_h * p.out_w;
  const int64_t ring = (int64_t)MfmaCfg::kDirectStages * c.bn() * 32;
  const int64_t stride = (cpad / 32) * 16 + 16;
  int images = 1;
  int64_t rows;
  if (ohow * 2 <= bm) {
    rows = (int64_t)(p.out_h - 1) * d.stride_height + (int64_t)(d.filter_height - 1) * d.dilation_height + 1;
    images = (int)std::min<int64_t>(bm / ohow, (lds_budget - ring) / std::max<int64_t>(1, rows * wp * stride));
    if (images < 1) return false;
  } else {
    const int rows_out = std::min(p.out_h, (bm + p.out_w - 2) / p.out_w + 1);
    rows = (int64_t)(rows_out - 1) * d.stride_height + (int64_t)(d.filter_height - 1) * d.dilation_height + 1;
  }
  int64_t bytes = ((int64_t)images * rows * wp * stride + 1023) / 1024 * 1024;
  int tx = 0;
  int64_t wh = wp;
  if (ohow * 2 > bm && tile_tx != nullptr) {
    const int th = bm / 32, tw = 32;
    const int64_t rows2 = (int64_t)(th - 1) * d.stride_height + (int64_t)(d.filter_height - 1) * d.dilation_height + 1;
    const int64_t wh2 = (int64_t)(tw - 1) * d.stride_width + (int64_t)(d.filter_width - 1) * d.dilation_width + 1;
    const int64_t bytes2 = (rows2 * wh2 * stride + 1023) / 1024 * 1024;
    const int ty_n = ceil_div(p.out_h, th), tx_n = ceil_div(p.out_w, tw);
    const double pad_strip = (double)ceil_div(ohow, bm) * bm / ohow, pad_2d = (double)ty_n * tx_n * bm / ohow;
    const bool strip_fits = bytes + ring <= lds_budget;
    const bool rule = pad_2d <= pad_strip + 0.03 && (!strip_fits || bytes2 * 10 <= bytes * 7);
    if (bytes2 + ring <= lds_budget && p.tile2d_pref != 2 && (rule || p.tile2d_pref == 1)) {
      tx = tx_n;
      rows = rows2;
      wh = wh2;
      bytes = bytes2;
      *tpi = ty_n * tx_n;
    }
  }
  if (bytes + ring > lds_budget) return false;
  if (tx == 0) *tpi = ohow * 2 <= bm ? 1 : ceil_div(ohow, bm);
  *halo_rows = (int)rows;
  *ps = (int)stride;
  *halo_bytes = (int)bytes;
  *ipt = images;
  if (tile_tx) *tile_tx = tx;
  if (halo_w) *halo_w = (int)wh;
  return true;
}

bool choose_direct_cfg(const HostPlan& p, MfmaCfg* out) {
  const int ohow = p.out_h * p.out_w;
  const bool wide = p.d.channels_out > 128 && (int64_t)p.d.batch * ceil_div(ohow, 128) >= 4096;
  int bn = wide ? 256 : p.d.channels_out > 64 ? 128 : 64;
  while (bn > 64 && p.d.groups > 1 && p.npg % bn) bn /= 2;
  struct Cand { const MfmaCfg* c; double padded; int64_t blocks; };
  Cand cand[2];
  int n = 0;
  for (int bm : {256, 128}) {
    if (bm == 256 && bn == 256) continue;
    const MfmaCfg* c = mfma_cfg_by_tile(bm, bn);
    int tpi, rows, ps, bytes, ipt, ttx, hw;
    if (!c || !direct_geometry(p, *c, &tpi, &rows, &ps, &bytes, &ipt, kDirectLdsAuto, &ttx, &hw)) continue;
    const double padded = ohow * 2 <= bm ? (double)bm / ((double)ipt * ohow) : (double)tpi * bm / (double)ohow;
    if (padded > 1.0 / 0.7) continue;
    const int64_t blocks = (int64_t)(ohow * 2 <= bm ? ceil_div(p.d.batch, ipt) : p.d.batch * tpi) * ceil_div(p.d.channels_out, bn);
    cand[n++] = Cand{c, padded, blocks};
  }
  if (n == 0) return false;
  int pick = 0;
  if (n == 2 && cand[0].c->bm() == 256 && (cand[0].padded - cand[1].padded > 0.08 || cand[0].blocks < 512)) pick = 1;
  *out = *cand[pick].c;
  return true;
}

size_t mfma_workspace_bytes(const HostPlan& p, int batch_chunk) {
  return (size_t)batch_chunk * p.hp * p.wp * (p.cpad / 2);
}

MfmaArgs make_mfma_args(const HostPlan& p, int batch_chunk) {
  const lce_hip_bconv2d_desc& d = p.d;
  MfmaArgs G{};
  G.H = d.in_height; G.W = d.in_width; G.Cw = p.cw; G.Cin = d.channels_in;
  G.Hp = p.hp; G.Wp = p.wp; G.PH = p.pad_h; G.PW = p.pad_w;
  G.NPIX = (uint32_t)((int64_t)batch_chunk * p.hp * p.wp); G.CPW = p.cpad / 32; G.KCH = p.d.groups > 1 ? group_chunks(p.d) : p.cpad / 64;
  G.Npad = p.npad;
  G.zero_border = p.zero_pad_mode == kZeroPadExact ? 1 : 0;
  G.x_bytes = (uint32_t)mfma_workspace_bytes(p, batch_chunk);
  G.w_bytes = (uint32_t)p.wq.size();
  G.div_npix = make_fastdiv(G.NPIX);
  G.div_wp = make_fastdiv((uint32_t)G.Wp);
  G.div_hp = make_fastdiv((uint32_t)G.Hp);
  G.div_npg = make_fastdiv((uint32_t)p.npg);
  G.a_bt = (float)p.backtransform_add;
  G.cmin = (float)p.clamp_min;
  G.cmax = (float)p.clamp_max;
  G.noclamp = (p.clamp_min <= 0 && (int64_t)p.clamp_max >= 2 * (int64_t)p.backtransform_add) ? 1 : 0;
  G.bit_thr = p.bit_thr;
  {
    const int lds = p.use_direct ? p.mfma.direct_lds_bytes(p.halo_bytes) : p.mfma.lds_bytes();
    const bool room = (p.mfma.threads() / 64) * p.mfma.wn * 4096 <= lds;
    G.i8_wide = (p.d.dst_type == LCE_HIP_I8 && p.d.channels_out % 16 == 0 && room) ? 1 : 0;
    G.f32_wide = (p.d.dst_type == LCE_HIP_F32 && p.d.channels_out % 4 == 0 && room &&
                  p.zero_pad_mode != kZeroPadCorrection) ? 1 : 0;
    if (p.epilogue_pref == 1) { G.f32_wide = 0; G.i8_wide = 0; }
  }
  if (p.use_direct) {
    G.TPI = p.tpi; G.OHOW = p.out_h * p.out_w; G.halo_rows = p.halo_rows; G.PS = p.ps;
    G.halo_bytes = p.halo_bytes; G.QG = (G.CPW + 3) / 4;
    G.Wh = p.halo_w; G.TX = p.tile_tx;
    G.IPT = p.ipt; G.B = batch_chunk; G.HPIX = p.halo_rows * p.halo_w;
    G.div_wh = make_fastdiv((uint32_t)G.Wh);
    G.div_tx = make_fastdiv((uint32_t)(G.TX > 0 ? G.TX : 1));
    G.div_tpi = make_fastdiv((uint32_t)G.TPI);
    G.div_qg = make_fastdiv((uint32_t)G.QG);
    G.div_ohow = make_fastdiv((uint32_t)G.OHOW);
    G.div_hpix = make_fastdiv((uint32_t)G.HPIX);
  }
  return G;
}

enum class Family { kNone, kStream, kWstream, kBlockGemm };
struct FamilyChoice {
  Family take = Family::kNone;
  StreamPick pick;
  double us = -1.0;
  std::string refusal;
};

static std::vector<StreamPick> stream_candidates(const HostPlan& p, const PlanOptions& o) {
  const int rows_pref = o.stream_rows_pref, il_pref = o.stream_interleave_pref, occ_pref = o.stream_occ_pref;
  std::vector<StreamPick> cands;
  if (il_pref <= 0) cands.push_back(StreamPick{rows_pref, 0});
  if (il_pref != 0)
    for (int r = p.out_h - 1; r >= 2; --r) {
      if (p.out_h % r != 0 || (rows_pref != 0 && rows_pref != r)) continue;
      const int px = r * p.out_w;
      if (rows_pref == 0 && ceil_div(px, 32) * 32 * 100 > px * 115) continue;
      cands.push_back(StreamPick{r, 1});
    }
  if (il_pref == 1 && cands.empty()) cands.push_back(StreamPick{rows_pref, 1});
  if (occ_pref == 2 || (occ_pref == 0 && stream_blocks_per_cu_max(p) >= 2)) {
    const size_t n1 = cands.size();
    for (size_t i = 0; i < n1; ++i) { cands.push_back(cands[i]); cands.back().occ = 2; }
    if (occ_pref == 2) cands.erase(cands.begin(), cands.begin() + (long)n1);
  }
  return cands;
}

static bool price_stream_pick(HostPlan& p, int batch_chunk, StreamPick& c, std::string* first_err) {
  c.us = -1.0;
  const std::string err = plan_stream(p, batch_chunk, c);
  if (!err.empty()) { if (first_err->empty()) *first_err = err; return false; }
  if (c.interleave && p.st_gstr <= 1) return false;
  c.us = estimate_stream_us(p, batch_chunk);
  return true;
}

static FamilyChoice price_stream_family(HostPlan& p, const PlanOptions& o, int64_t pixels, int batch_chunk) {
  FamilyChoice r;
  if (!stream_supported(p)) { r.refusal = plan_stream(p, 1, StreamPick{}); return r; }
  std::vector<StreamPick> cands = stream_candidates(p, o);
  int best = -1;
  auto price_from = [&](size_t first) {
    for (size_t i = first; i < cands.size(); ++i)
      if (price_stream_pick(p, batch_chunk, cands[i], &r.refusal) && (best < 0 || cands[i].us < cands[best].us)) best = (int)i;
  };
  price_from(0);
  if (best < 0 && o.stream_interleave_pref == 1) {
    cands.push_back(StreamPick{o.stream_rows_pref, 0, o.stream_occ_pref == 2 ? 2 : 1});
    price_from(cands.size() - 1);
  }
  if (best >= 0) { r.take = Family::kStream; r.pick = cands[best]; r.us = cands[best].us; }
  else if (r.refusal.empty()) r.refusal = "bconv2d: the streaming kernel cannot run this launch";
  double best_us = best >= 0 ? r.us : 1e30;
  const bool debug = p.dbg_level >= 1;
  if (debug)
    for (const StreamPick& c : cands)
      fprintf(stderr, "[lce plan] stream rows=%d il=%d blocks/CU=%d: %.2f us\n", c.rows, c.interleave, c.occ, c.us);
  if (!auto_rule(o)) return r;
  if (wstream_supported(p) && !p.dbg_no_wstream && plan_wstream(p, batch_chunk).empty()) {
    const double us = estimate_wstream_us(p, batch_chunk);
    if (debug) fprintf(stderr, "[lce plan] wstream images=%d blocks=%d: %.2f us\n", p.ws_ipb, p.ws_nb, us);
    if (us < best_us) { best_us = r.us = us; r.take = Family::kWstream; }
  }
  const double gemm_us = estimate_block_gemm_us(p, pixels);
  if (debug) fprintf(stderr, "[lce plan] block GEMM: %.2f us\n", gemm_us);
  if (gemm_us < best_us) r.take = Family::kBlockGemm;
  return r;
}

static FamilyChoice plan_forced_wstream(HostPlan& p, int batch_chunk) {
  FamilyChoice r;
  r.refusal = plan_wstream(p, batch_chunk);
  if (r.refusal.empty()) { r.take = Family::kWstream; r.us = estimate_wstream_us(p, batch_chunk); }
  return r;
}

static std::string commit_stream_family(HostPlan& p, const FamilyChoice& c, int batch_chunk) {
  const lce_hip_bconv2d_desc& d = p.d;
  const bool wstream = c.take == Family::kWstream;
  p.est_us = c.us;
  if (!wstream) {
    const std::string err = plan_stream(p, batch_chunk, c.pick);
    if (!err.empty()) return err;
  }
  const MfmaCfg want = *mfma_cfg_by_tile(128, 64);
  const int layout = wstream ? 1 : 0;
  const bool repack = p.wq.empty() || p.mfma.bn() != want.bn() || p.wq_layout != layout || p.kch != stream_chunks(d);
  p.wq_layout = layout;
  p.mfma = want;
  p.use_mfma = true;
  p.use_wstream = wstream;
  p.use_stream = !wstream;
  p.use_tiled = false;
  p.cpad = stream_chunks(d) * 64;
  p.npad = ceil_div(d.channels_out, 64) * 64;
  p.hp = (int)padded_height(p);
  if (repack && p.have_weights) pack_for_mfma(p);
  char nm[96];
  if (wstream) {
    snprintf(nm, sizeof nm, "bconv2d_wstream<%s,3x3x%d,images%d,blocks%d>", dst_name(d), 64 * stream_chunks(d), p.ws_ipb, p.ws_nb);
  } else {
    char ph[40] = "";
    if ((4 >> p.st_pph_log) < std::min(4, ceil_div(d.channels_out, 64))) snprintf(ph, sizeof ph, ",phases%d", 1 << p.st_pph_log);
    if (p.st_nstrip > 1) snprintf(ph + strlen(ph), sizeof ph - strlen(ph), ",strips%d", p.st_wso);
    if (p.st_gstr > 1) snprintf(ph + strlen(ph), sizeof ph - strlen(ph), ",il");
    if (p.st_occ > 1) snprintf(ph + strlen(ph), sizeof ph - strlen(ph), ",x%d", p.st_occ);
    snprintf(nm, sizeof nm, "bconv2d_stream<%s,3x3x%d,rows%d%s>", dst_name(d), 64 * stream_chunks(d), p.st_rs, ph);
  }
  p.kernel_name = nm;
  return "";
}

static std::string choose_gemm_tile(const HostPlan& p, const PlanOptions& o, int64_t pixels, MfmaCfg* want, bool* direct) {
  const lce_hip_bconv2d_desc& d = p.d;
  *want = choose_mfma_cfg(p, pixels);
  *direct = false;
  if (o.engine_pref >= kEngineMfma && o.tile_pref.tm != 0) {
    const MfmaCfg* forced = mfma_cfg_by_tile(o.tile_pref.tm, o.tile_pref.tn);
    if (!forced) return "bconv2d: no matrix-core kernel instance for the requested block tile";
    if (d.groups > 1 && p.npg % forced->bn())
      return "bconv2d: the requested block tile would straddle channel groups";
    *want = *forced;
    *direct = o.engine_pref == kEngineDirect;
  } else if (o.engine_pref != kEngineMfma) {
    MfmaCfg dc;
    const int ks_deep = d.filter_height * d.filter_width * ceil_div(d.channels_in / std::max(1, d.groups), 64);
    auto tiny_deep = [&](const MfmaCfg& c) {
      return o.engine_pref == kEngineAuto && ks_deep >= 27 && ((pixels + c.bm() - 1) / c.bm()) * ceil_div(d.channels_out, c.bn()) <= 128;
    };
    if (choose_direct_cfg(p, &dc) && !tiny_deep(dc)) {
      *want = dc;
      *direct = true;
    } else if (o.engine_pref == kEngineDirect) {
      for (int bm : {128, 256}) {
        const MfmaCfg* c = mfma_cfg_by_tile(bm, d.channels_out > 64 && (d.groups == 1 || p.npg % 128 == 0) ? 128 : 64);
        int a, b, c2, e, f, ttx, hw;
        if (c && direct_geometry(p, *c, &a, &b, &c2, &e, &f, kDirectLdsMax, &ttx, &hw)) { *want = *c; break; }
      }
      *direct = true;
    }
  }
  return "";
}

static std::string select_block_gemm(HostPlan& p, const PlanOptions& o, int64_t pixels) {
  const lce_hip_bconv2d_desc& d = p.d;
  p.use_mfma = true;
  p.use_tiled = false;
  p.est_us = estimate_block_gemm_us(p, pixels);
  MfmaCfg want;
  bool direct;
  const std::string err = choose_gemm_tile(p, o, pixels, &want, &direct);
  if (!err.empty()) return err;
  const bool repack = p.wq.empty() || p.mfma.bn() != want.bn() || p.wq_layout != 0 ||
                      p.kch != (d.groups > 1 ? group_chunks(d) : ceil_div(d.channels_in, 64));
  p.wq_layout = 0;
  p.mfma = want;
  p.cpad = ceil_div(d.channels_in, 64) * 64;
  p.npad = ceil_div(d.channels_out, want.bn()) * want.bn();
  p.hp = (int)padded_height(p);
  p.wp = (int)padded_width(p);
  if (repack && p.have_weights) pack_for_mfma(p);
  if (direct) {
    if (!direct_geometry(p, want, &p.tpi, &p.halo_rows, &p.ps, &p.halo_bytes, &p.ipt,
                         o.engine_pref == kEngineDirect ? kDirectLdsMax : kDirectLdsAuto, &p.tile_tx, &p.halo_w))
      return "bconv2d: the direct matrix-core variant cannot hold this tile's input halo in LDS";
    p.use_direct = true;
  }
  char nm[96];
  if (!direct) { p.tile_tx = 0; p.halo_w = p.wp; }
  snprintf(nm, sizeof nm, "bconv2d_mfma%s<%s,%dx%d>%s", p.use_direct ? "_direct" : "", dst_name(d), want.bm(), want.bn(),
           p.use_direct && p.tile_tx > 0 ? "/2d" : "");
  p.kernel_name = nm;
  if ((o.engine_pref == kEnginePointwise || auto_rule(o)) && pointwise_supported(p, pixels, &p.pw_nc, &p.pw_nj) &&
      (o.engine_pref == kEnginePointwise || pointwise_preferred(p, pixels))) {
    p.use_pointwise = true;
    snprintf(nm, sizeof nm, "bconv2d_pointwise<%s,K%dx64,N%dx32%s>", dst_name(d), p.pw_nc, p.pw_nj,
             d.stride_height != 1 || d.stride_width != 1 ? ",strided" : "");
    p.kernel_name = nm;
  }
  return "";
}

static std::string choose_valu_tile(const HostPlan& p, const PlanOptions& o, int64_t pixels, TileShape* chosen) {
  const bool bp = p.d.dst_type == LCE_HIP_BITPACKED;
  *chosen = TileShape{0, 0};
  if (o.kernel_pref == kKernelGeneral) return "";
  if (o.tile_pref.tm != 0) {
    if (tiled_supports(p, o.tile_pref.tn)) *chosen = o.tile_pref;
    else if (o.kernel_pref == kKernelTiled) return "bconv2d: the requested tile cannot run this convolution";
  } else {
    const TileShape order_f[] = {{1, 32}, {1, 16}, {2, 16}, {2, 32}, {4, 16}};
    const TileShape order_b[] = {{1, 32}, {2, 32}};
    const TileShape* order = bp ? order_b : order_f;
    const int count = bp ? 2 : 5;
    for (int k = 0; k < count && chosen->tm == 0; ++k) {
      const TileShape t = order[k];
      if (!tiled_supports(p, t.tn)) continue;
      const int64_t tasks = ((pixels + 64 * t.tm - 1) / (64 * t.tm)) * ceil_div(p.d.channels_out, t.tn);
      if (!bp && k == 0 && tasks < 32768 && tiled_supports(p, 16)) continue;
      *chosen = t;
    }
    for (int k = count - 1; k >= 0 && chosen->tm == 0; --k)
      if (tiled_supports(p, order[k].tn)) *chosen = order[k];
  }
  if (chosen->tm == 0 && o.kernel_pref == kKernelTiled)
    return "bconv2d: the tiled kernel cannot run this convolution (grouped, channels per group "
           "not a multiple of the tile)";
  return "";
}

static std::string select_valu(HostPlan& p, const PlanOptions& o, int64_t pixels) {
  const lce_hip_bconv2d_desc& d = p.d;
  TileShape chosen;
  const std::string err = choose_valu_tile(p, o, pixels, &chosen);
  if (!err.empty()) return err;
  char name[96];
  if (chosen.tm != 0) {
    const bool repack = !p.use_tiled || p.tile.tn != chosen.tn || p.packed.empty();
    p.use_tiled = true;
    p.tile = chosen;
    if (repack && p.have_weights) pack_for_tile(p);
    p.nt = ceil_div(d.channels_out, chosen.tn);
    snprintf(name, sizeof name, "bconv2d_tiled<%s,TM=%d,TN=%d,CH=%d>", dst_name(d), chosen.tm, chosen.tn, p.ch);
  } else {
    p.use_tiled = false;
    p.tile = TileShape{0, 0};
    snprintf(name, sizeof name, "bconv2d_general<%s>", dst_name(d));
  }
  p.kernel_name = name;
  return "";
}

std::string select_kernel(HostPlan& p, int64_t pixels) {
  const PlanOptions& o = p;
  const lce_hip_bconv2d_desc& d = p.d;
  p.ch = (p.cwg % 4 == 0) ? 4 : (p.cwg % 2 == 0) ? 2 : 1;
  p.use_mfma = false;
  p.use_direct = false;
  p.use_pointwise = false;
  if (o.engine_pref == kEnginePointwise && !pointwise_supported(p, pixels, &p.pw_nc, &p.pw_nj))
    return "bconv2d: the pointwise kernel runs 1x1 ungrouped convolutions with 64, 128, 256 or 512 input channels (after padding to 64) "
           "and a multiple of 32 output channels (pointwise_channels must divide them)";
  if (o.engine_pref >= kEngineMfma && !mfma_supported(p))
    return "bconv2d: the matrix-core engine cannot run this convolution (channels per group not a multiple of 64, or too deep)";
  p.use_stream = false;
  p.use_wstream = false;
  p.est_us = -1.0;
  const int batch_chunk = images_per_launch(p, pixels);
  FamilyChoice family;
  if (o.engine_pref == kEngineWstream) family = plan_forced_wstream(p, batch_chunk);
  else if (o.engine_pref == kEngineStream || auto_rule(o)) family = price_stream_family(p, o, pixels, batch_chunk);
  std::string err;
  if (family.take == Family::kStream || family.take == Family::kWstream) {
    err = commit_stream_family(p, family, batch_chunk);
  } else if (o.engine_pref == kEngineStream || o.engine_pref == kEngineWstream) {
    err = family.refusal;
  } else if (o.engine_pref >= kEngineMfma ||
             (auto_rule(o) && mfma_supported(p) && (family.take == Family::kBlockGemm || pixels * d.channels_out >= (1 << 16)))) {
    err = select_block_gemm(p, o, pixels);
  } else {
    err = select_valu(p, o, pixels);
  }
  if (err.empty() && d.dst_type == LCE_HIP_I8 && p.use_mfma && p.have_weights && !p.wq.empty()) prepare_int8_epilogue(p);
  return err;
}

int max_batch_per_launch(const HostPlan& p) {
  const int64_t per_image_bytes = (int64_t)p.d.in_height * p.d.in_width * p.cw * 4;
  const int64_t per_image_pixels = (int64_t)p.out_h * p.out_w;
  int64_t by_bytes = ((1ll << 31) - 1) / per_image_bytes;
  int64_t by_pixels = ((1ll << 31) - 64 * 4 - 1) / per_image_pixels;
  int64_t b = std::min(by_bytes, by_pixels);
  if (p.engine_pref != kEngineValu && mfma_supported(p)) {
    const int cpad = ceil_div(p.d.channels_in, 64) * 64;
    b = std::min<int64_t>(b, (int64_t)(((1ll << 31) - 1) / (padded_height(p) * padded_width(p) * (cpad / 2))));
    b = std::min<int64_t>(b, ((1ll << 31) - 1) / std::max<int64_t>(1, out_bytes_of(p, 1)));
  }
  b = std::max<int64_t>(1, std::min<int64_t>(b, p.d.batch));
  return (int)b;
}

ConvArgs make_conv_args(const HostPlan& p, int batch_chunk) {
  const lce_hip_bconv2d_desc& d = p.d;
  ConvArgs A{};
  A.H = d.in_height; A.W = d.in_width; A.Cw = p.cw; A.Cwg = p.cwg;
  A.OH = p.out_h; A.OW = p.out_w; A.N = d.channels_out; A.Npg = p.npg;
  A.KH = d.filter_height; A.KW = d.filter_width;
  A.SH = d.stride_height; A.SW = d.stride_width;
  A.DH = d.dilation_height; A.DW = d.dilation_width;
  A.PH = p.pad_h; A.PW = p.pad_w;
  A.M = batch_chunk * p.out_h * p.out_w;
  A.NT = p.nt;
  A.PT = p.use_tiled ? (A.M + 64 * p.tile.tm - 1) / (64 * p.tile.tm) : 0;
  A.Wout = p.wout;
  A.in_bytes = (uint32_t)((int64_t)batch_chunk * d.in_height * d.in_width * p.cw * 4);
  A.div_ow = make_fastdiv((uint32_t)p.out_w);
  A.div_oh = make_fastdiv((uint32_t)p.out_h);
  A.clamp_min = p.clamp_min; A.clamp_max = p.clamp_max;
  A.zero_pad_mode = p.zero_pad_mode;
  A.bzp = (d.channels_in / d.groups) / 2;
  A.eKH = (d.filter_height - 1) * d.dilation_height + 1;
  A.eKW = (d.filter_width - 1) * d.dilation_width + 1;
  A.left_off = ((p.out_w - 1) * d.stride_width + A.eKW - d.in_width) / 2;
  A.top_off = ((p.out_h - 1) * d.stride_height + A.eKH - d.in_height) / 2;
  return A;
}

}
```

compute-engine_amd/csrc/lce_plan.h:

```cpp
#pragma once
#include <stdint.h>

#include <algorithm>
#include <string>
#include <vector>

#include "../../include/lce_hip.h"
#include "lce_kernel_args.h"

namespace lce {

struct TileShape {
  int tm, tn;
};

struct MfmaCfg {
  int wgm, wgn, wm, wn;
  int bm() const { return 32 * wm * wgm; }
  int bn() const { return 32 * wn * wgn; }
  int threads() const { return 64 * wgm * wgn; }
  static constexpr int kStages = 4;
  static constexpr int kDirectStages = 3;
  int epilogue_scratch_bytes() const { return (threads() / 64) * wn * 4096; }
  int lds_bytes() const { return std::max(kStages * (bm() + bn()) * 32, epilogue_scratch_bytes()); }
  int direct_lds_bytes(int halo_bytes) const {
    return std::max(halo_bytes + kDirectStages * bn() * 32, epilogue_scratch_bytes());
  }
};
const MfmaCfg* mfma_cfg_by_tile(int bm, int bn);

enum EnginePref {
  kEngineAuto = 0,
  kEngineValu,
  kEngineMfma,
  kEngineDirect,
  kEnginePointwise,
  kEngineStream,
  kEngineWstream,
};
enum KernelPref { kKernelAuto = 0, kKernelTiled, kKernelGeneral };

struct PlanOptions {
  int engine_pref = kEngineAuto;
  int kernel_pref = kKernelAuto;
  TileShape tile_pref{0, 0};
  int tile2d_pref = 0;
  int phase = 0;
  int epilogue_pref = 0;
  int pw_tiles_pref = 0;
  int pw_nj_pref = 0;
  bool int8_exact_pref = false;
  int stream_rows_pref = 0;
  int stream_noflat = 0;
  int stream_phases_pref = 0;
  int stream_strip_pref = -1;
  int stream_interleave_pref = -1;
  int stream_occ_pref = 0;
  int ws_blocks_pref = 0, ws_images_pref = 0;
  bool cus_forced = false;
};

enum : unsigned {
  kStaleSelection = 1,
  kStaleUpload = 2,
  kStalePacked = 4,
  kStaleWeightImage = 8,
};

struct HostPlan : PlanOptions {
  lce_hip_bconv2d_desc d{};
  int out_h = 0, out_w = 0, pad_h = 0, pad_w = 0;
  int cw = 0, cwg = 0, npg = 0, wout = 0;
  int backtransform_add = 0;
  int zero_pad_mode = kZeroPadNone;

  bool have_weights = false;
  bool want_sign = false;
  std::vector<float> mul, bias;
  int32_t clamp_min = 0, clamp_max = 0;
  float bit_thr = 0.0f;
  std::vector<int32_t> thresholds;
  std::vector<uint32_t> filter;
  std::vector<float> zero_pad_cache;

  bool use_tiled = false;
  TileShape tile{0, 0};
  int ch = 1;
  int nt = 0;
  std::string kernel_name;

  bool use_direct = false;
  int tpi = 0, halo_rows = 0, ps = 0, halo_bytes = 0, ipt = 1;
  int tile_tx = 0, halo_w = 0;
  bool use_mfma = false;
  bool use_pointwise = false;
  int pw_nc = 0, pw_nj = 0;
  MfmaCfg mfma{0, 0, 0, 0};
  int cpad = 0, hp = 0, wp = 0, npad = 0;
  int kch = 0;
  bool int8_floor_ok = false;
  int int8_bias_adjusted = 0;
  std::vector<uint8_t> wq;
  int wq_layout = 0;
  std::vector<float> mul_q, bias_q, thr_q;

  bool use_stream = false;
  int num_cus = 256;
  int st_rs = 0, st_spi = 0, st_srs = 0, st_pbs = 0, st_pph_log = 0, st_ny = 1, st_qg = 0, st_ipr = 0;
  int st_pitch = 0;
  int st_nstrip = 1, st_rseg = 0, st_wso = 0;
  int st_gstr = 1;
  int st_occ = 1;
  int st_flat = 0;
  int st_nq = 0;
  int st_spb = 0, st_gx = 0, st_rows = 0, st_ring_bytes = 0, st_batch = 0;
  std::vector<uint32_t> st_tabs;
  uint32_t st_tab_lim = 0, st_tab_ctx = 0, st_tab_sgn = 0, st_tab_seg = 0;

  bool use_wstream = false;
  int ws_ipb = 0, ws_parts = 0, ws_nq = 0, ws_npxg = 0, ws_nb = 0, ws_ny = 1;
  int ws_hp = 0, ws_wp = 0, ws_pitch = 0, ws_img_pitch = 0, ws_qg = 0, ws_lds_images = 0;
  int ws_occupancy = 1;
  uint32_t ws_tab_part = 0, ws_tab_ctx = 0;
  int64_t ws_cost = 0;

  double est_us = -1.0;

  int dbg_level = 0;
  bool dbg_no_wstream = false;
  bool dbg_int8_exact = false;
  bool dbg_int8_full = false;

  std::vector<uint32_t> packed;
  std::vector<float> mul_p, bias_p;
  std::vector<int32_t> thr_p;
  std::vector<int32_t> oob_corr;
};

std::string validate_and_infer(HostPlan& p);

std::string set_plan_option(HostPlan& p, const char* key, const char* value, unsigned* invalidates);

inline bool int8_forms_kernel(const HostPlan& p) { return p.use_mfma && (p.use_stream || p.use_wstream || p.use_pointwise); }
inline bool int8_one_instruction_forms(const HostPlan& p) { return int8_forms_kernel(p) && p.int8_floor_ok; }

void fold_parameters(HostPlan& p, const int32_t* filter_ohwi, const float* post_mul,
                     const float* post_bias, const int32_t* thresholds);

float int8_below_threshold(int32_t zero_point);

bool tiled_supports(const HostPlan& p, int tn);

std::string select_kernel(HostPlan& p, int64_t pixels);

int max_batch_per_launch(const HostPlan& p);

bool mfma_supported(const HostPlan& p);
bool choose_direct_cfg(const HostPlan& p, MfmaCfg* out);
constexpr int kDirectLdsMax = 160 * 1024;
constexpr int kDirectLdsAuto = 80 * 1024;
bool direct_geometry(const HostPlan& p, const MfmaCfg& c, int* tpi, int* halo_rows, int* ps, int* halo_bytes,
                     int* ipt, int lds_budget, int* tile_tx = nullptr, int* halo_w = nullptr);
MfmaArgs make_mfma_args(const HostPlan& p, int batch_chunk);
bool pointwise_supported(const HostPlan& p, int64_t pixels, int* nc, int* nj);
inline int pointwise_bank_steps(int chunks) { return chunks <= 2 ? chunks : chunks <= 4 ? 4 : chunks == 8 ? 8 : 0; }
constexpr int64_t pw_small_launch_tiles = 16384;
PwArgs make_pw_args(const HostPlan& p, int batch_chunk);
size_t mfma_workspace_bytes(const HostPlan& p, int batch_chunk);

ConvArgs make_conv_args(const HostPlan& p, int batch_chunk);

bool stream_supported(const HostPlan& p);
struct StreamPick {
  int rows = 0;
  int interleave = 0;
  int occ = 1;
  double us = 0.0;
};
std::string plan_stream(HostPlan& p, int batch_chunk, const StreamPick& pick);
StreamArgs make_stream_args(const HostPlan& p, int batch_chunk);
bool wstream_supported(const HostPlan& p);
std::string plan_wstream(HostPlan& p, int batch_chunk);
WsArgs make_ws_args(const HostPlan& p, int batch_chunk);
constexpr int kWsLdsExtra = 4 * 8192;
inline int wstream_lds_bytes(const HostPlan& p) { return p.ws_lds_images + kWsLdsExtra; }
constexpr int kStreamLdsExtra = 4 * 8192 + 4096;
constexpr int kStreamLdsExtraKsplit = 4 * 4096 + 4096 + 4 * 8192;
inline int stream_chunks(const lce_hip_bconv2d_desc& d) {
  const int c = (d.channels_in + 63) / 64;
  return c <= 2 ? c : c <= 4 ? 4 : c <= 8 ? 8 : 0;
}
inline bool stream_ksplit(const HostPlan& p) { return stream_chunks(p.d) > 4; }
inline int stream_lds_extra(const HostPlan& p) {
  if (stream_ksplit(p)) return kStreamLdsExtraKsplit;
  if (p.d.dst_type == LCE_HIP_BITPACKED && stream_chunks(p.d) == 1) return 2048;
  return (p.d.dst_type == LCE_HIP_BITPACKED ? 4096 : kStreamLdsExtra) + 1024;
}
inline int stream_blocks_per_cu_max(const HostPlan& p) {
  return p.d.dst_type == LCE_HIP_BITPACKED && stream_chunks(p.d) == 1 ? 2 : 1;
}
inline int stream_lds_bytes(const HostPlan& p) { return p.st_ring_bytes + stream_lds_extra(p); }

}
```

compute-engine_amd/csrc/lce_plan_stream.cpp:

```cpp
#include "lce_plan.h"
#include "lce_plan_internal.h"

#include <limits.h>
#include <string.h>

#include <algorithm>
#include <cmath>
#include <cstdio>
#include <cstdlib>

namespace lce {

bool stream_supported(const HostPlan& p) {
  const lce_hip_bconv2d_desc& d = p.d;
  if (!mfma_supported(p) || d.groups != 1) return false;
  if (d.filter_height != 3 || d.filter_width != 3) return false;
  if (d.dilation_height != 1 || d.dilation_width != 1) return false;
  if (p.zero_pad_mode == kZeroPadCorrection) return false;
  if (d.dst_type == LCE_HIP_F32 && d.channels_out % 4) return false;
  if (d.dst_type == LCE_HIP_I8 && d.channels_out % 16) return false;
  const int kch = stream_chunks(d);
  return kch == 1 || kch == 2 || kch == 4 || kch == 8;
}

static bool simulate_stream(const HostPlan& p, int rs, int spb, int pph_log, bool flat, int ow, int in_w, int* ring_rows,
                            std::vector<uint32_t>* sched) {
  const lce_hip_bconv2d_desc& d = p.d;
  const int kh = d.filter_height, sh = d.stride_height;
  const int srs = (rs - 1) * sh + kh, pbs = ceil_div(rs * ow, 32);
  const int cpw = stream_chunks(d) * 2, qg = ceil_div(cpw, 4);
  const int64_t ipr = (int64_t)in_w * qg;
  const int pph = 1 << pph_log;
  const int64_t npx = (int64_t)rs * ow;
  const int64_t nblk = flat ? (spb * npx + 31) / 32 : (int64_t)spb * pbs;
  const int64_t usteps = (nblk + pph - 1) / pph, ntile = (usteps + 3) / 4;
  const int64_t total = (int64_t)spb * srs * ipr;
  if (ntile < 1 || total >= (1ll << 31) || ntile > (1 << 20)) return false;
  std::vector<int64_t> need(ntile + 2), first(ntile);
  for (int64_t t = 0; t < ntile; ++t) {
    int64_t hi = 0, lo = INT64_MAX;
    for (int64_t q = 4 * t * pph; q < std::min<int64_t>(nblk, 4 * (t + 1) * pph); ++q) {
      if (flat) {
        const int64_t p0 = q * 32, p1 = std::min<int64_t>(q * 32 + 31, spb * npx - 1);
        lo = std::min(lo, (p0 / npx) * srs + (p0 % npx) / ow * sh);
        hi = std::max(hi, (p1 / npx) * srs + (p1 % npx) / ow * sh + kh - 1);
        continue;
      }
      const int64_t gl = q / pbs, pb = q % pbs;
      const int64_t r_first = std::min<int64_t>(pb * 32 / ow, rs - 1), r_last = std::min<int64_t>((pb * 32 + 31) / ow, rs - 1);
      lo = std::min(lo, gl * srs + r_first * sh);
      hi = std::max(hi, gl * srs + r_last * sh + kh - 1);
    }
    need[t] = std::min(total, (hi + 1) * ipr);
    first[t] = lo;
  }
  need[ntile] = need[ntile + 1] = need[ntile - 1];
  for (int64_t t = 1; t < ntile; ++t) need[t] = std::max(need[t], need[t - 1]);
  const int64_t cap = stream_ksplit(p) ? 768 : 512;
  std::vector<int64_t> m(ntile + 2), s(ntile + 2);
  m[ntile + 1] = m[ntile] = need[ntile];
  for (int64_t t = ntile - 1; t >= 0; --t) m[t] = std::max(need[t], m[t + 1] - cap);
  s[0] = m[0];
  for (int64_t t = 0; t <= ntile; ++t) {
    int64_t inc = 0;
    while (s[t] + inc < m[t + 1]) inc += 256;
    s[t + 1] = std::min(total, s[t] + inc);
    if (s[t + 1] < m[t + 1] || inc > cap) return false;
  }
  int64_t rows = kh;
  for (int64_t t = 0; t < ntile; ++t)
    if (s[t + 1] > 0) rows = std::max(rows, (s[t + 1] - 1) / ipr - first[t] + 1);
  *ring_rows = (int)rows;
  sched->resize(ntile + 2);
  for (int64_t t = 0; t < ntile + 2; ++t) (*sched)[t] = (uint32_t)s[t];
  return true;
}

static bool plan_stream_geometry(HostPlan& p, int batch_chunk, const StreamPick& pick, int wso, std::string* why);

std::string plan_stream(HostPlan& p, int batch_chunk, const StreamPick& pick) {
  const lce_hip_bconv2d_desc& d = p.d;
  if (!stream_supported(p))
    return "bconv2d: the streaming kernel runs ungrouped 3x3 convolutions without dilation, with at most 512 input "
           "channels (on its 64-, 128-, 256- or 512-channel instance) and whole 16-byte groups of output channels (float: a multiple of 4, "
           "int8: of 16), and not the SAME-zero correction semantics";
  if (pick.occ == 2 && stream_blocks_per_cu_max(p) < 2)
    return "bconv2d: stream_blocks_per_cu=2: only the bitpacked-output instance of the 64-input-channel bank is compiled for two blocks per CU";
  const uint32_t row_bytes = stream_row_bytes(p);
  if ((int64_t)batch_chunk * p.out_h * p.out_w * row_bytes >= (1ll << 31))
    return "bconv2d: the streaming kernel binds the whole output of a launch to one buffer resource (< 2 GiB)";
  std::vector<int> widths;
  if (p.stream_strip_pref <= 0) widths.push_back(0);
  if (p.stream_strip_pref > 0 && stream_chunks(d) != 4)
    return "bconv2d: stream_strip: column strips exist for the 256-channel filter bank only (193..256 input channels)";
  if (stream_chunks(d) == 4 && p.stream_strip_pref != 0) {
    if (p.stream_strip_pref > 0) {
      if (p.stream_strip_pref % 32 != 0 || p.out_w % p.stream_strip_pref != 0)
        return "bconv2d: stream_strip must be a multiple of 32 that divides the output width";
      widths.push_back(p.stream_strip_pref);
    } else if (p.out_w % 32 == 0 && p.out_w > 64) {
      if (p.out_w % 64 == 0) widths.push_back(64);
      widths.push_back(32);
    }
  }
  std::string why = pick.occ == 2 ? "bconv2d: stream_blocks_per_cu=2: two blocks' row rings do not fit a CU's LDS for this layer"
                                           : "bconv2d: the streaming kernel's row ring does not fit LDS for this layer";
  for (int wso : widths)
    if (plan_stream_geometry(p, batch_chunk, pick, wso, &why)) return "";
  return why;
}

static bool plan_stream_geometry(HostPlan& p, int batch_chunk, const StreamPick& pick, int wso, std::string* why) {
  const lce_hip_bconv2d_desc& d = p.d;
  const uint32_t row_bytes = stream_row_bytes(p);
  const bool strips = wso > 0;
  const int nstrip = strips ? p.out_w / wso : 1;
  const int ow_seg = strips ? wso : p.out_w;
  const int in_w_seg = strips ? (wso - 1) * d.stride_width + d.filter_width : d.in_width;
  const int nsl = ceil_div(d.channels_out, 64);
  int pph_log = nsl >= 3 ? 0 : nsl == 2 ? 1 : 2;
  if (p.stream_phases_pref > 0) pph_log = std::max(pph_log, p.stream_phases_pref == 4 ? 2 : p.stream_phases_pref == 2 ? 1 : 0);
  const bool ksplit = stream_ksplit(p);
  if (ksplit) pph_log = 0;
  const int nslb = ksplit ? 2 : 4 >> pph_log, ny = ceil_div(nsl, nslb), pph = 1 << pph_log;
  const int wp = strips ? in_w_seg : (int)padded_width(p);
  const int kch = stream_chunks(d), ps = kch * 32 + 16;
  int skew16 = 0;
  if (d.stride_height % 2 == 1 && !strips) {
    const int want = (int)(((int64_t)p.out_w * d.stride_width * (ps / 16)) % 16);
    for (int k = 0; k < 16; ++k)
      if (((int64_t)d.stride_height * ((int64_t)wp * (ps / 16) + k)) % 16 == want) { skew16 = k; break; }
  }
#ifdef LCE_STREAM_NO_SKEW
  skew16 = 0;
#endif
  const int pitch = wp * ps + skew16 * 16;
  const int occ = !strips && pick.occ == 2 && stream_blocks_per_cu_max(p) >= 2 ? 2 : 1;
  const int cus = std::max(1, p.num_cus * occ / ny);
  auto run_length = [&](int rseg) -> int64_t {
    const int64_t s = (int64_t)batch_chunk * nstrip * rseg, gx = std::min<int64_t>(s, cus);
    const int64_t spb = (s + gx - 1) / gx;
    return strips ? std::min<int64_t>(spb, 128) : spb;
  };
  struct Cand { int rs; int64_t cost; };
  std::vector<Cand> cands;
  for (int rs = p.out_h; rs >= 1; --rs) {
    if (p.out_h % rs) continue;
    if (pick.rows > 0 && rs != pick.rows) continue;
    const int64_t spb = run_length(p.out_h / rs), s = (int64_t)batch_chunk * nstrip * (p.out_h / rs);
    const bool flat_c = !strips && rs == p.out_h && spb > 1 && (rs * p.out_w) % 32 != 0 && !p.stream_noflat && ksplit;
    const int64_t blocks = flat_c ? (spb * rs * p.out_w + 31) / 32 : spb * ceil_div(rs * ow_seg, 32);
    const int64_t rounds = (ceil_div((int)s, (int)spb) + cus - 1) / cus;
    const int64_t steps = (blocks + pph - 1) / pph;
    cands.push_back(Cand{rs, (steps + 4) * rounds * 4096 + (strips ? std::abs(rs - 14) : 0)});
  }
  if (cands.empty()) { *why = "bconv2d: stream_rows must divide the output height"; return false; }
  std::stable_sort(cands.begin(), cands.end(), [](const Cand& a, const Cand& b) { return a.cost < b.cost; });
  for (const Cand& c : cands) {
    const int rs = c.rs, rseg = p.out_h / rs, spi = nstrip * rseg;
    const int64_t s = (int64_t)batch_chunk * spi, spb = run_length(rseg);
    int rows = 0;
    std::vector<uint32_t> sched;
    const bool flat = !strips && rs == p.out_h && spb > 1 && (rs * p.out_w) % 32 != 0 && !p.stream_noflat && ksplit;
    if (!simulate_stream(p, rs, (int)spb, pph_log, flat, ow_seg, in_w_seg, &rows, &sched)) continue;
    const int64_t ring = ((int64_t)rows * pitch + 1023) / 1024 * 1024;
    if ((ring + stream_lds_extra(p)) * occ > 160 * 1024) continue;
    p.st_occ = occ;
    const int pbs = ceil_div(rs * ow_seg, 32);
    if (strips && (rs * ow_seg) % 32 != 0) continue;
    const int64_t nq = flat ? (spb * (int64_t)rs * p.out_w + 31) / 32 : spb * pbs;
    p.st_flat = flat ? 1 : 0;
    p.st_nq = (int)nq;
    const int64_t gx_plan = ceil_div((int)s, (int)spb);
    const int64_t gstr = (pick.interleave > 0 && !flat && spb > 1) ? gx_plan : 1;
    p.st_gstr = (int)gstr;
    if (nq * 1024 > (64ll << 20)) continue;
    p.st_rs = rs; p.st_spi = spi; p.st_srs = (rs - 1) * d.stride_height + d.filter_height;
    p.st_pbs = pbs; p.st_pph_log = pph_log; p.st_ny = ny;
    p.st_qg = ceil_div(kch * 2, 4); p.st_ipr = in_w_seg * p.st_qg;
    p.st_nstrip = nstrip; p.st_rseg = rseg; p.st_wso = ow_seg;
    p.st_spb = (int)spb; p.st_gx = (int)ceil_div((int)s, (int)spb); p.st_rows = rows; p.st_ring_bytes = (int)ring;
    p.st_batch = batch_chunk;
    p.wp = wp;
    if (p.dbg_level >= 2)
      fprintf(stderr,
              "[lce plan] stream geometry: rows/segment %d, ring %d rows x %d B = %lld B (+%d), blocks %d x %d, segments/block %lld\n",
              rs, rows, pitch, (long long)ring, stream_lds_extra(p), p.st_gx, ny, (long long)spb);
    p.st_pitch = pitch;
    const size_t n_sched = (sched.size() + 3) / 4 * 4, n_lim = ((size_t)nq + 3) / 4 * 4;
    const size_t n_sgn = d.dst_type == LCE_HIP_BITPACKED ? 0 : (size_t)nq * 64;
    const size_t n_seg = strips ? ((size_t)nq + 3) / 4 * 4 : 0;
    p.st_tab_lim = (uint32_t)(n_sched * 4);
    p.st_tab_ctx = (uint32_t)((n_sched + n_lim) * 4);
    p.st_tab_sgn = (uint32_t)((n_sched + n_lim + (size_t)nq * 256) * 4);
    p.st_tab_seg = (uint32_t)((n_sched + n_lim + (size_t)nq * 256 + n_sgn) * 4);
    p.st_tabs.assign(n_sched + n_lim + (size_t)nq * 256 + n_sgn + n_seg, 0u);
    std::copy(sched.begin(), sched.end(), p.st_tabs.begin());
    for (size_t i = sched.size(); i < n_sched; ++i) p.st_tabs[i] = sched.back();
    const int npx = rs * ow_seg, sh = d.stride_height, sw = d.stride_width;
    const int64_t total_px = spb * (int64_t)npx;
    const bool ragged = flat ? total_px % 32 != 0 : npx % 32 != 0;
    const int lpr = d.dst_type == LCE_HIP_F32 ? (ksplit ? 8 : 16) : d.dst_type == LCE_HIP_I8 ? (ksplit ? 2 : 4) : 0;
    for (int64_t q = 0; q < nq; ++q) {
      const int64_t gl = flat ? 0 : q / pbs, pb = flat ? q : q % pbs;
      const int64_t seg_px = flat ? total_px : npx;
      const bool partial = ragged && (flat ? q == nq - 1 : pb == pbs - 1);
      p.st_tabs[n_sched + q] = (uint32_t)std::min<int64_t>(31, seg_px - pb * 32 - 1);
      for (int lane = 0; lane < 64; ++lane) {
        const int l31 = lane & 31, half = lane >> 5;
        int64_t pix = std::min<int64_t>(pb * 32 + l31, seg_px - 1);
        const int64_t sg_ = flat ? pix / npx : gl;
        if (flat) pix %= npx;
        const int64_t r = pix / ow_seg, ox = pix % ow_seg;
        const int64_t s0 = sg_ * p.st_srs + r * sh;
        uint32_t* e = &p.st_tabs[n_sched + n_lim + ((size_t)q * 64 + lane) * 4];
        for (int fy = 0; fy < 3; ++fy)
          e[fy] = (uint32_t)(((s0 + fy) % rows) * pitch + ox * sw * ps + half * 16);
        const int rowl = lpr ? lane / lpr : l31;
        const int64_t blk_px = strips ? ((pb * 32) / ow_seg) * (int64_t)p.out_w + (pb * 32) % ow_seg : gl * gstr * npx + pb * 32;
        e[3] = (uint32_t)((blk_px + rowl) * (int64_t)row_bytes);
        if (partial) e[3] |= 0x80000000u;
        if (strips) p.st_tabs[n_sched + n_lim + (size_t)nq * 256 + n_sgn + q] = (uint32_t)gl;
        if (n_sgn) {
          uint32_t& sg = p.st_tabs[n_sched + n_lim + (size_t)nq * 256 + (size_t)q * 64 + lane];
          sg = (uint32_t)((blk_px + l31) * (int64_t)p.wout * 4);
          if (partial) sg |= 0x80000000u;
        }
      }
    }
    return true;
  }
  return false;
}

StreamArgs make_stream_args(const HostPlan& p, int batch_chunk) {
  const lce_hip_bconv2d_desc& d = p.d;
  StreamArgs G{};
  G.H = d.in_height; G.W = d.in_width; G.Cw = p.cw; G.Cin = d.channels_in;
  G.OH = p.out_h; G.OW = p.out_w; G.N = d.channels_out; G.Npad = p.npad; G.Wout = p.wout;
  G.SH = d.stride_height; G.SW = d.stride_width; G.PH = p.pad_h;
  G.PW = p.st_nstrip > 1 ? 0 : p.pad_w;
  G.NSTRIP = p.st_nstrip; G.RSEG = p.st_rseg; G.WSo = p.st_wso; G.XS0 = p.pad_w;
  G.B = batch_chunk;
  G.Wp = p.wp; G.pitch = p.st_pitch; G.R = p.st_rows; G.ring_bytes = p.st_ring_bytes;
  G.zero_border = p.zero_pad_mode == kZeroPadExact ? 1 : 0;
  G.QG = p.st_qg; G.IPR = p.st_ipr; G.RS = p.st_rs; G.SPI = p.st_spi; G.SRS = p.st_srs; G.PBS = p.st_pbs;
  G.S = batch_chunk * p.st_spi;
  const int gx = std::min(G.S, std::max(1, p.num_cus * p.st_occ / p.st_ny));
  G.SPB = std::min(p.st_spb, ceil_div(G.S, std::max(1, gx)));
  if (p.st_flat) G.SPB = p.st_spb;
  G.GSTR = 1; G.G0M = G.SPB; G.GX = ceil_div(G.S, std::max(1, G.SPB));
  if (p.st_gstr > 1) {
    G.GSTR = p.st_gstr; G.G0M = 1; G.SPB = p.st_spb; G.GX = std::min(G.S, p.st_gstr);
  }
  G.pph_log = p.st_pph_log;
  G.flat = p.st_flat;
  G.NPX = p.st_rs * p.out_w;
  G.NQ = p.st_nq;
  G.need0 = p.st_tabs.empty() ? 0u : p.st_tabs[0];
  G.in_bytes = (uint32_t)((int64_t)batch_chunk * d.in_height * d.in_width * p.cw * 4);
  G.w_bytes = (uint32_t)p.wq.size();
  G.out_bytes = (uint32_t)((int64_t)batch_chunk * p.out_h * p.out_w * stream_row_bytes(p));
  G.tab_bytes = (uint32_t)(p.st_tabs.size() * 4);
  G.tab_lim = p.st_tab_lim;
  G.tab_ctx = p.st_tab_ctx;
  G.tab_sgn = p.st_tab_sgn;
  G.tab_seg = p.st_tab_seg;
  G.sign_bytes = (uint32_t)((int64_t)batch_chunk * p.out_h * p.out_w * p.wout * 4);
  G.bit_thr = p.bit_thr;
  G.a_bt = (float)p.backtransform_add;
  G.cmin = (float)p.clamp_min;
  G.cmax = (float)p.clamp_max;
  G.div_ipr = make_fastdiv_nb((uint32_t)G.IPR);
  G.div_qg = make_fastdiv_nb((uint32_t)G.QG);
  G.div_srs = make_fastdiv_nb((uint32_t)G.SRS);
  G.div_spi = make_fastdiv_nb((uint32_t)G.SPI);
  G.div_r = make_fastdiv_nb((uint32_t)G.R);
  G.div_rseg = make_fastdiv_nb((uint32_t)std::max(1, G.RSEG));
  G.div_gstr = make_fastdiv_nb((uint32_t)G.GSTR);
  return G;
}


bool wstream_supported(const HostPlan& p) {
  if (!stream_supported(p)) return false;
  const int kch = stream_chunks(p.d);
  return kch == 2 || kch == 4 || kch == 8;
}

static int64_t wstream_cost(int64_t blocks, int cus, int occupancy, const std::vector<int>& nb_of_block, int ks, int items_per_lane) {
  std::vector<int64_t> load(cus, 0);
  int64_t worst = 0, last_nb = 0;
  for (int64_t b = 0; b < blocks; ++b) {
    load[b % cus] += nb_of_block[b];
    worst = std::max(worst, load[b % cus]);
  }
  for (int64_t b = std::max<int64_t>(0, blocks - cus); b < blocks; ++b) last_nb = std::max<int64_t>(last_nb, nb_of_block[b]);
  const int64_t rounds = (blocks + (int64_t)cus * occupancy - 1) / ((int64_t)cus * occupancy);
  const int64_t prologue = 2200 + 300 * items_per_lane, epilogue = 450 * last_nb;
  return worst * ks * 2 * 34 + rounds * prologue + epilogue + (occupancy < 2 ? (blocks + cus - 1) / cus * (prologue + epilogue) : 0);
}

std::string plan_wstream(HostPlan& p, int batch_chunk) {
  const lce_hip_bconv2d_desc& d = p.d;
  if (!wstream_supported(p))
    return "bconv2d: the weight-streaming kernel runs ungrouped 3x3 convolutions without dilation over 65 .. 512 input channels "
           "(on its 128-, 256- or 512-channel instance) and whole 16-byte groups of output channels (float: a multiple of 4, int8: of 16), "
           "and not the SAME-zero correction semantics";
  if ((int64_t)batch_chunk * p.out_h * p.out_w * stream_row_bytes(p) >= (1ll << 31))
    return "bconv2d: the weight-streaming kernel binds the whole output of a launch to one buffer resource (< 2 GiB)";
  const int kch = stream_chunks(d), ps = kch * 32 + 16, ks = 9 * kch;
  const int hp = (p.out_h - 1) * d.stride_height + d.filter_height, wp = (p.out_w - 1) * d.stride_width + d.filter_width;
  int skew16 = 0;
  if (d.stride_height % 2 == 1) {
    const int want = (int)(((int64_t)p.out_w * d.stride_width * (ps / 16)) % 16);
    for (int k = 0; k < 16; ++k)
      if (((int64_t)d.stride_height * ((int64_t)wp * (ps / 16) + k)) % 16 == want) { skew16 = k; break; }
  }
  const int pitch = wp * ps + skew16 * 16, img_pitch = hp * pitch;
  const int qg = ceil_div(kch * 2, 4), ohw = p.out_h * p.out_w;
  const int ny = ceil_div(ceil_div(d.channels_out, 64), 4), cus = std::max(1, p.num_cus);
  int best_ipb = 0;
  int64_t best_cost = 0;
  const int nbmax = p.ws_blocks_pref > 0 ? p.ws_blocks_pref : 4;
  for (int ipb = 1; ipb <= std::min(batch_chunk, 64); ++ipb) {
    if (p.ws_images_pref > 0 && ipb != p.ws_images_pref) continue;
    const int64_t lds_images = ((int64_t)ipb * img_pitch + 1023) / 1024 * 1024;
    if (lds_images + kWsLdsExtra > 160 * 1024) break;
    const int occupancy = (int)std::min<int64_t>(2, (160 * 1024) / (lds_images + kWsLdsExtra));
    const int nq = ceil_div(ipb * ohw, 32), parts = ceil_div(nq, nbmax), groups = ceil_div(batch_chunk, ipb);
    std::vector<int> nb_of_block;
    for (int y = 0; y < ny; ++y)
      for (int part = 0; part < parts; ++part)
        for (int g = 0; g < groups; ++g) nb_of_block.push_back(nq / parts + (part < nq % parts ? 1 : 0));
    const int items_per_lane = ceil_div(ipb * hp * wp * qg, 256);
    const int64_t cost = wstream_cost((int64_t)nb_of_block.size(), cus, occupancy, nb_of_block, ks, items_per_lane);
    if (best_ipb == 0 || cost < best_cost) { best_ipb = ipb; best_cost = cost; }
  }
  if (best_ipb == 0) return "bconv2d: one image of this layer does not fit the weight-streaming kernel's LDS (whole images are resident)";
  const int ipb = best_ipb;
  const int nq = ceil_div(ipb * ohw, 32), parts = ceil_div(nq, nbmax);
  p.ws_ipb = ipb; p.ws_parts = parts; p.ws_nq = nq; p.ws_npxg = ipb * ohw; p.ws_nb = ceil_div(nq, parts); p.ws_ny = ny;
  p.ws_hp = hp; p.ws_wp = wp; p.ws_pitch = pitch; p.ws_img_pitch = img_pitch; p.ws_qg = qg;
  p.ws_lds_images = (int)(((int64_t)ipb * img_pitch + 1023) / 1024 * 1024);
  p.ws_occupancy = (int)std::min<int64_t>(2, (160 * 1024) / (p.ws_lds_images + kWsLdsExtra));
  p.ws_cost = best_cost;
  p.st_batch = batch_chunk;
  const size_t n_part = ((size_t)parts * 2 + 3) / 4 * 4;
  p.ws_tab_part = 0;
  p.ws_tab_ctx = (uint32_t)(n_part * 4);
  p.st_tabs.assign(n_part + (size_t)nq * 256, 0u);
  int q0 = 0;
  for (int part = 0; part < parts; ++part) {
    const int nb = nq / parts + (part < nq % parts ? 1 : 0);
    p.st_tabs[2 * part] = (uint32_t)q0;
    p.st_tabs[2 * part + 1] = (uint32_t)nb;
    q0 += nb;
  }
  for (int q = 0; q < nq; ++q)
    for (int lane = 0; lane < 64; ++lane) {
      const int l31 = lane & 31, half = lane >> 5;
      const int pix = std::min(q * 32 + l31, ipb * ohw - 1);
      const int img = pix / ohw, oy = (pix % ohw) / p.out_w, ox = pix % p.out_w;
      uint32_t* e = &p.st_tabs[n_part + ((size_t)q * 64 + lane) * 4];
      for (int fy = 0; fy < 3; ++fy)
        e[fy] = (uint32_t)((int64_t)img * img_pitch + (int64_t)(oy * d.stride_height + fy) * pitch + (int64_t)ox * d.stride_width * ps +
                           half * 16);
    }
  return "";
}

WsArgs make_ws_args(const HostPlan& p, int batch_chunk) {
  const lce_hip_bconv2d_desc& d = p.d;
  WsArgs G{};
  G.H = d.in_height; G.W = d.in_width; G.Cw = p.cw; G.Cin = d.channels_in;
  G.OH = p.out_h; G.OW = p.out_w; G.N = d.channels_out; G.Npad = p.npad; G.Wout = p.wout;
  G.SH = d.stride_height; G.SW = d.stride_width; G.PH = p.pad_h; G.PW = p.pad_w;
  G.B = batch_chunk;
  G.IPB = p.ws_ipb; G.GROUPS = ceil_div(batch_chunk, p.ws_ipb); G.PARTS = p.ws_parts;
  G.NPXG = p.ws_npxg; G.NQ = p.ws_nq;
  G.Hp = p.ws_hp; G.Wp = p.ws_wp; G.pitch = p.ws_pitch; G.img_pitch = p.ws_img_pitch;
  G.QG = p.ws_qg; G.items = p.ws_ipb * p.ws_hp * p.ws_wp * p.ws_qg;
  G.zero_border = p.zero_pad_mode == kZeroPadExact ? 1 : 0;
  G.noclamp = (p.clamp_min <= 0 && p.clamp_max >= 2 * p.backtransform_add) ? 1 : 0;
  G.lds_images = (uint32_t)p.ws_lds_images;
  G.in_bytes = (uint32_t)((int64_t)batch_chunk * d.in_height * d.in_width * p.cw * 4);
  G.w_bytes = (uint32_t)p.wq.size();
  G.out_bytes = (uint32_t)((int64_t)batch_chunk * p.out_h * p.out_w * stream_row_bytes(p));
  G.sign_bytes = (uint32_t)((int64_t)batch_chunk * p.out_h * p.out_w * p.wout * 4);
  G.tab_bytes = (uint32_t)(p.st_tabs.size() * 4);
  G.tab_part = p.ws_tab_part;
  G.tab_ctx = p.ws_tab_ctx;
  G.a_bt = (float)p.backtransform_add;
  G.cmin = (float)p.clamp_min;
  G.cmax = (float)p.clamp_max;
  G.bit_thr = p.bit_thr;
  G.div_qg = make_fastdiv_nb((uint32_t)G.QG);
  G.div_wp = make_fastdiv_nb((uint32_t)G.Wp);
  G.div_hp = make_fastdiv_nb((uint32_t)G.Hp);
  G.div_groups = make_fastdiv_nb((uint32_t)G.GROUPS);
  return G;
}

}
```

Baseline: 2672000 billion.

## Add eight-block-step tile variant to the streaming bconv kernel

```diff
diff --git a/compute-engine_amd/csrc/lce_dispatch_stream.h b/compute-engine_amd/csrc/lce_dispatch_stream.h
--- a/compute-engine_amd/csrc/lce_dispatch_stream.h
+++ b/compute-engine_amd/csrc/lce_dispatch_stream.h
@@ -21,8 +21,21 @@
 stream_fn stream_by_fast(int kch, bool fast, bool strips) {
   return fast ? stream_by_kch<DST, true, CLAMP, SIGN, I8F>(kch, strips) : stream_by_kch<DST, false, CLAMP, SIGN, I8F>(kch, strips);
 }
+template <int DST, bool CLAMP, bool SIGN>
+stream_fn stream_tile8(int kch, bool fast, bool strips) {
+  if constexpr (DST == kDstFloat) {
+    if (kch == 4 && !strips)
+      return fast ? bconv2d_stream<kDstFloat, 3, 3, 4, true, CLAMP, SIGN, false, false, false, 8>
+                  : bconv2d_stream<kDstFloat, 3, 3, 4, false, CLAMP, SIGN, false, false, false, 8>;
+  }
+  return nullptr;
+}
 template <int DST, bool CLAMP, bool I8F>
 stream_fn find_stream_part(int kch, bool fast, bool sign, bool strips) {
+  if (kch & kStreamKeyTile8) {
+    const int chunks = kch & ~kStreamKeyTile8;
+    return sign ? stream_tile8<DST, CLAMP, true>(chunks, fast, strips) : stream_tile8<DST, CLAMP, false>(chunks, fast, strips);
+  }
   if constexpr (DST == kDstBitpacked) return stream_by_fast<kDstBitpacked, false, false>(kch, fast, strips);
   else return sign ? stream_by_fast<DST, CLAMP, true, I8F>(kch, fast, strips) : stream_by_fast<DST, CLAMP, false, I8F>(kch, fast, strips);
 }
diff --git a/compute-engine_amd/csrc/lce_kernel_args.h b/compute-engine_amd/csrc/lce_kernel_args.h
--- a/compute-engine_amd/csrc/lce_kernel_args.h
+++ b/compute-engine_amd/csrc/lce_kernel_args.h
@@ -135,6 +135,7 @@
   int32_t flat;
   int32_t NPX;
   int32_t NQ;
+  int32_t TS;
   uint32_t need0;
   uint32_t in_bytes, w_bytes, out_bytes;
   uint32_t tab_bytes, tab_lim, tab_ctx, tab_sgn;
diff --git a/compute-engine_amd/csrc/lce_kernel_types.h b/compute-engine_amd/csrc/lce_kernel_types.h
--- a/compute-engine_amd/csrc/lce_kernel_types.h
+++ b/compute-engine_amd/csrc/lce_kernel_types.h
@@ -29,16 +29,23 @@
 }
 int launch_expand_fp4(unsigned grid_x, void* stream, const uint32_t* in, void* workspace, const MfmaArgs& G, uint64_t chunks);
 pointwise_fn lookup_pointwise(int dst, int nc, int nj, bool strided, bool i8_floor);
+constexpr int kStreamKeyTile8 = 0x100;
+struct StreamForm {
+  bool fast;
+  int tile_steps;
+};
 stream_fn lookup_stream_f32(int kch, bool fast, bool sign, bool strips);
 stream_fn lookup_stream_f32_clamp(int kch, bool fast, bool sign, bool strips);
 stream_fn lookup_stream_i8(int kch, bool fast, bool sign, bool strips);
 stream_fn lookup_stream_i8_floor(int kch, bool fast, bool sign, bool strips);
 stream_fn lookup_stream_bitpacked(int kch, bool fast, bool strips);
-inline stream_fn lookup_stream(int dst, int kch, bool fast, bool clamp, bool sign, bool strips, bool i8_floor) {
+inline stream_fn lookup_stream(int dst, int kch, StreamForm form, bool clamp, bool sign, bool strips, bool i8_floor) {
+  if (form.tile_steps != 4 && form.tile_steps != 8) return nullptr;
+  const int key = kch | (form.tile_steps == 8 ? kStreamKeyTile8 : 0);
   switch (dst) {
-    case LCE_HIP_F32: return clamp ? lookup_stream_f32_clamp(kch, fast, sign, strips) : lookup_stream_f32(kch, fast, sign, strips);
-    case LCE_HIP_I8: return i8_floor ? lookup_stream_i8_floor(kch, fast, sign, strips) : lookup_stream_i8(kch, fast, sign, strips);
-    default: return lookup_stream_bitpacked(kch, fast, strips);
+    case LCE_HIP_F32: return clamp ? lookup_stream_f32_clamp(key, form.fast, sign, strips) : lookup_stream_f32(key, form.fast, sign, strips);
+    case LCE_HIP_I8: return i8_floor ? lookup_stream_i8_floor(key, form.fast, sign, strips) : lookup_stream_i8(key, form.fast, sign, strips);
+    default: return lookup_stream_bitpacked(key, form.fast, strips);
   }
 }
 wstream_fn lookup_wstream_f32(int kch, int nb, bool sign);
@@ -56,8 +63,8 @@
 int mfma_selftest_pointwise();
 int mfma_selftest_stream();
 
-inline bool stream_fast(const StreamArgs& G) {
-  return (G.Cin == 64 || G.Cin == 128 || G.Cin == 256 || G.Cin == 512) && !G.zero_border;
+inline StreamForm stream_fast(const StreamArgs& G) {
+  return StreamForm{(G.Cin == 64 || G.Cin == 128 || G.Cin == 256 || G.Cin == 512) && !G.zero_border, G.TS};
 }
 inline bool stream_clamps(const StreamArgs& G) { return !(G.cmin <= 0.0f && G.cmax >= 2.0f * G.a_bt); }
 
diff --git a/compute-engine_amd/csrc/lce_kernels_stream.h b/compute-engine_amd/csrc/lce_kernels_stream.h
--- a/compute-engine_amd/csrc/lce_kernels_stream.h
+++ b/compute-engine_amd/csrc/lce_kernels_stream.h
@@ -19,12 +19,13 @@
 constexpr int stream_blocks_per_cu(int dst, int kch, bool ksplit, bool strips) {
   return dst == kDstBitpacked && kch == 1 && !ksplit && !strips ? 2 : 1;
 }
-template <int DST, int KH, int KW, int KCH, bool FAST, bool CLAMP, bool SIGN, bool KSPLIT = false, bool STRIPS = false, bool I8F = false>
+template <int DST, int KH, int KW, int KCH, bool FAST, bool CLAMP, bool SIGN, bool KSPLIT = false, bool STRIPS = false, bool I8F = false, int TS = 4>
 LCE_KERNEL void __launch_bounds__(256, stream_blocks_per_cu(DST, KCH, KSPLIT, STRIPS))
 bconv2d_stream(const StreamArgs G, const uint8_t* __restrict__ xin, const uint8_t* __restrict__ wq,
                const float* __restrict__ mul, const float* __restrict__ bias, const float* __restrict__ thrf,
                const uint32_t* __restrict__ tabs, void* __restrict__ out, uint32_t* __restrict__ sign_words) {
   static_assert(!SIGN || DST != kDstBitpacked, "a bitpacked-output plan already writes bits");
+  static_assert(TS == 4 || (TS == 8 && !KSPLIT), "tile steps of four block steps, or of eight (one woven item, used twice)");
   constexpr int KCHW = KSPLIT ? KCH / 2 : KCH;
   constexpr bool FLATC = KSPLIT;
   constexpr int KS = KH * KW * KCHW;
@@ -66,7 +67,7 @@
   int dyn_lim = nseg * G.NPX - (nblk_all - 1) * 32 - 1;
   keep_in_vgpr(dyn_last);
   keep_in_vgpr(dyn_lim);
-  const int ntile = (usteps + 3) >> 2;
+  const int ntile = TS == 4 || usteps <= 4 ? (usteps + 3) >> 2 : 1 + ((usteps + 3) >> 3);
   const uint32_t* const sched = tabs;
   const rsrc_t rtab = make_rsrc(tabs, G.tab_bytes);
 
@@ -272,7 +273,8 @@
     for (int k = 0; k < 4; ++k) item_write(wv0[k], dv0[k], mv0[k]);
   }
   LCE_SPH(61);
-  constexpr uint32_t kItemB = KSPLIT ? 512u : 256u;
+  constexpr uint32_t kItemB0 = KSPLIT ? 512u : 256u;
+  constexpr uint32_t kItemB = TS == 8 ? 512u : kItemB0;
   u32x4 pwa, pwb = {0u, 0u, 0u, 0u}, pwc = {0u, 0u, 0u, 0u};
   uint32_t pda, pdb = dump, pdc = dump;
   int pma, pmb = 0, pmc = 0;
@@ -281,8 +283,8 @@
     const uint32_t a = sched[0], b = sched[1];
     item_issue(a + (uint32_t)tid, b, pwa, pda, pma);
     if constexpr (KSPLIT) item_issue(a + (uint32_t)(256 + tid), b, pwc, pdc, pmc);
-    have_b = b - a > kItemB;
-    if (have_b) item_issue(a + kItemB + (uint32_t)tid, b, pwb, pdb, pmb);
+    have_b = b - a > kItemB0;
+    if (have_b) item_issue(a + kItemB0 + (uint32_t)tid, b, pwb, pdb, pmb);
   }
   auto bank_home = [&](auto ksc) LCE_LAMBDA_INLINE {
     constexpr int ks = decltype(ksc)::value;
@@ -607,8 +609,9 @@
   uint32_t next_ob = kOobOffset, next_sob = kOobOffset, epi_sob = kOobOffset;
   bool next_part = false;
   Issue isa, isc;
-  auto step = [&](auto kc_, auto first_, int u, uint32_t sch1, uint32_t sch2) LCE_LAMBDA_INLINE {
-    constexpr int k = decltype(kc_)::value, PAR = k & 1;
+  constexpr int kProdNone = 0, kProdExpand = 1, kProdIssue = 2;
+  auto step = [&](auto kc_, auto first_, auto nst_, auto prod_, int u, uint32_t e0, uint32_t e1) LCE_LAMBDA_INLINE {
+    constexpr int k = decltype(kc_)::value, PAR = k & 1, NST = decltype(nst_)::value, PROD = decltype(prod_)::value;
     constexpr bool FIRST = decltype(first_)::value != 0;
     static_assert(!FIRST || k == 0, "the first block step is step 0 of tile step 0");
     if constexpr (k == 0) {
@@ -631,7 +634,7 @@
           if constexpr (g + 1 < NG) {
             if constexpr ((g + 1) * GA + d1 < KS) af[fs ^ 1][d1] = *(const u32x4*)(lds0 + frag_addr(cur, (g + 1) * GA + d1));
             if constexpr ((g + 1) * GA + d0 < KS) af[fs ^ 1][d0] = *(const u32x4*)(lds0 + frag_addr(cur, (g + 1) * GA + d0));
-          } else if constexpr (k < 3) {
+          } else if constexpr (k < NST - 1) {
             af[fs ^ 1][d1] = *(const u32x4*)(lds0 + frag_addr(nxt, d1));
             af[fs ^ 1][d0] = *(const u32x4*)(lds0 + frag_addr(nxt, d0));
             if constexpr (KS - (NG - 1) * GA < 2) {
@@ -704,18 +707,18 @@
         if constexpr (KSPLIT && ks == (NG - 1) * GA - 1) ctx_khalf(nxt);
 #ifndef LCE_ST_NOPROD
         if constexpr (ks > SA) {
-          if constexpr (k == 0) {
+          if constexpr (PROD == kProdExpand) {
             constexpr int lo = stream_unit_lo(16, ks - SA - 1, NPG), hi = stream_unit_lo(16, ks - SA, NPG);
             if constexpr (lo + 0 < hi) write_chunk(IntC<lo + 0>{}, pwa, pda, pma);
             if constexpr (lo + 1 < hi) write_chunk(IntC<lo + 1>{}, pwa, pda, pma);
             if constexpr (lo + 2 < hi) write_chunk(IntC<lo + 2>{}, pwa, pda, pma);
             if constexpr (lo + 3 < hi) write_chunk(IntC<lo + 3>{}, pwa, pda, pma);
             static_assert(hi - lo <= 4, "chunks per gap");
-          } else if constexpr (k == 1) {
+          } else if constexpr (PROD == kProdIssue) {
             constexpr int lo = stream_unit_lo(kIssueChunks, ks - SA - 1, NPG), hi = stream_unit_lo(kIssueChunks, ks - SA, NPG);
-            if constexpr (lo + 0 < hi) issue_chunk(IntC<lo + 0>{}, isa, sch1 + (uint32_t)tid, sch2, pwa, pda, pma);
-            if constexpr (lo + 1 < hi) issue_chunk(IntC<lo + 1>{}, isa, sch1 + (uint32_t)tid, sch2, pwa, pda, pma);
-            if constexpr (lo + 2 < hi) issue_chunk(IntC<lo + 2>{}, isa, sch1 + (uint32_t)tid, sch2, pwa, pda, pma);
+            if constexpr (lo + 0 < hi) issue_chunk(IntC<lo + 0>{}, isa, e0 + (uint32_t)tid, e1, pwa, pda, pma);
+            if constexpr (lo + 1 < hi) issue_chunk(IntC<lo + 1>{}, isa, e0 + (uint32_t)tid, e1, pwa, pda, pma);
+            if constexpr (lo + 2 < hi) issue_chunk(IntC<lo + 2>{}, isa, e0 + (uint32_t)tid, e1, pwa, pda, pma);
             static_assert(hi - lo <= 3, "chunks per gap");
           } else if constexpr (KSPLIT && k == 2) {
             constexpr int lo = stream_unit_lo(16, ks - SA - 1, NPG), hi = stream_unit_lo(16, ks - SA, NPG);
@@ -725,9 +728,9 @@
             if constexpr (lo + 3 < hi) write_chunk(IntC<lo + 3>{}, pwc, pdc, pmc);
           } else if constexpr (KSPLIT && k == 3) {
             constexpr int lo = stream_unit_lo(kIssueChunks, ks - SA - 1, NPG), hi = stream_unit_lo(kIssueChunks, ks - SA, NPG);
-            if constexpr (lo + 0 < hi) issue_chunk(IntC<lo + 0>{}, isc, sch1 + (uint32_t)(256 + tid), sch2, pwc, pdc, pmc);
-            if constexpr (lo + 1 < hi) issue_chunk(IntC<lo + 1>{}, isc, sch1 + (uint32_t)(256 + tid), sch2, pwc, pdc, pmc);
-            if constexpr (lo + 2 < hi) issue_chunk(IntC<lo + 2>{}, isc, sch1 + (uint32_t)(256 + tid), sch2, pwc, pdc, pmc);
+            if constexpr (lo + 0 < hi) issue_chunk(IntC<lo + 0>{}, isc, e0 + (uint32_t)(256 + tid), e1, pwc, pdc, pmc);
+            if constexpr (lo + 1 < hi) issue_chunk(IntC<lo + 1>{}, isc, e0 + (uint32_t)(256 + tid), e1, pwc, pdc, pmc);
+            if constexpr (lo + 2 < hi) issue_chunk(IntC<lo + 2>{}, isc, e0 + (uint32_t)(256 + tid), e1, pwc, pdc, pmc);
           }
         }
 #endif
@@ -754,17 +757,43 @@
 
   using TagFirst = IntC<1>;
   using TagSteady = IntC<0>;
-  auto tile_step = [&](auto first_, int T) LCE_LAMBDA_INLINE {
-    const uint32_t sch1 = sched[T + 1], sch2 = sched[T + 2];
-    step(IntC<0>{}, first_, 4 * T + 0, sch1, sch2);
-    if (4 * T + 1 < usteps) step(IntC<1>{}, TagSteady{}, 4 * T + 1, sch1, sch2);
-    if (4 * T + 2 < usteps) step(IntC<2>{}, TagSteady{}, 4 * T + 2, sch1, sch2);
-    if (4 * T + 3 < usteps) step(IntC<3>{}, TagSteady{}, 4 * T + 3, sch1, sch2);
+  using N4 = IntC<4>;
+  using N8 = IntC<8>;
+  using PNone = IntC<kProdNone>;
+  using PExpand = IntC<kProdExpand>;
+  using PIssue = IntC<kProdIssue>;
+  auto tile_end = [&](int T, uint32_t sch1, uint32_t sch2) LCE_LAMBDA_INLINE {
     if (have_b) item_write(pwb, pdb, pmb);
     have_b = sch2 - sch1 > kItemB;
     if (have_b) item_issue(sch1 + kItemB + (uint32_t)tid, sch2, pwb, pdb, pmb);
     block_barrier_keep_vm();
     LCE_SPH(2 + T);
+  };
+  auto tile_step = [&](auto first_, int T) LCE_LAMBDA_INLINE {
+    const uint32_t sch1 = sched[T + 1], sch2 = sched[T + 2];
+    if constexpr (TS == 4) {
+      step(IntC<0>{}, first_, N4{}, PExpand{}, 4 * T + 0, 0u, 0u);
+      if (4 * T + 1 < usteps) step(IntC<1>{}, TagSteady{}, N4{}, PIssue{}, 4 * T + 1, sch1, sch2);
+      if (4 * T + 2 < usteps) step(IntC<2>{}, TagSteady{}, N4{}, PNone{}, 4 * T + 2, 0u, 0u);
+      if (4 * T + 3 < usteps) step(IntC<3>{}, TagSteady{}, N4{}, PNone{}, 4 * T + 3, sch1, sch2);
+    } else if constexpr (decltype(first_)::value != 0) {
+      step(IntC<0>{}, first_, N4{}, PExpand{}, 0, 0u, 0u);
+      if (1 < usteps) step(IntC<1>{}, TagSteady{}, N4{}, PIssue{}, 1, sch1 + 256u, sch2);
+      if (2 < usteps) step(IntC<2>{}, TagSteady{}, N4{}, PNone{}, 2, 0u, 0u);
+      if (3 < usteps) step(IntC<3>{}, TagSteady{}, N4{}, PNone{}, 3, 0u, 0u);
+    } else {
+      const int u0 = 8 * T - 4;
+      const uint32_t sch0 = sched[T];
+      step(IntC<0>{}, first_, N8{}, PExpand{}, u0 + 0, 0u, 0u);
+      if (u0 + 1 < usteps) step(IntC<1>{}, TagSteady{}, N8{}, PIssue{}, u0 + 1, sch0, sch1);
+      if (u0 + 2 < usteps) step(IntC<2>{}, TagSteady{}, N8{}, PNone{}, u0 + 2, 0u, 0u);
+      if (u0 + 3 < usteps) step(IntC<3>{}, TagSteady{}, N8{}, PNone{}, u0 + 3, 0u, 0u);
+      if (u0 + 4 < usteps) step(IntC<4>{}, TagSteady{}, N8{}, PExpand{}, u0 + 4, 0u, 0u);
+      if (u0 + 5 < usteps) step(IntC<5>{}, TagSteady{}, N8{}, PIssue{}, u0 + 5, sch1 + 256u, sch2);
+      if (u0 + 6 < usteps) step(IntC<6>{}, TagSteady{}, N8{}, PNone{}, u0 + 6, 0u, 0u);
+      if (u0 + 7 < usteps) step(IntC<7>{}, TagSteady{}, N8{}, PNone{}, u0 + 7, 0u, 0u);
+    }
+    tile_end(T, sch1, sch2);
   };
   if (ntile > 0) tile_step(TagFirst{}, 0);
   for (int T = 1; T < ntile; ++T) tile_step(TagSteady{}, T);
diff --git a/compute-engine_amd/csrc/lce_plan.cpp b/compute-engine_amd/csrc/lce_plan.cpp
--- a/compute-engine_amd/csrc/lce_plan.cpp
+++ b/compute-engine_amd/csrc/lce_plan.cpp
@@ -146,6 +146,10 @@
   } else if (!strcmp(key, "stream_blocks_per_cu")) {
     if ((v = word_index(value, {"auto", "1", "2"})) < 0) return "plan_set_option: stream_blocks_per_cu must be auto, 1 or 2";
     o.stream_occ_pref = v;
+    stale = plan_and_upload;
+  } else if (!strcmp(key, "stream_tile_steps")) {
+    if (!int_value(value, &v) || !in_set(v, {0, 4, 8})) return "plan_set_option: stream_tile_steps must be 0 (auto), 4 or 8";
+    o.stream_tile_pref = v;
     stale = plan_and_upload;
   } else if (!strcmp(key, "stream_flat")) {
     if ((v = word_index(value, {"0", "1"})) < 0) return "plan_set_option: stream_flat must be 0 or 1";
@@ -821,6 +825,7 @@
     if (p.st_nstrip > 1) snprintf(ph + strlen(ph), sizeof ph - strlen(ph), ",strips%d", p.st_wso);
     if (p.st_gstr > 1) snprintf(ph + strlen(ph), sizeof ph - strlen(ph), ",il");
     if (p.st_occ > 1) snprintf(ph + strlen(ph), sizeof ph - strlen(ph), ",x%d", p.st_occ);
+    if (p.stream_tile_pref != 0) snprintf(ph + strlen(ph), sizeof ph - strlen(ph), ",t%d", p.st_tile_steps);
     snprintf(nm, sizeof nm, "bconv2d_stream<%s,3x3x%d,rows%d%s>", dst_name(d), 64 * stream_chunks(d), p.st_rs, ph);
   }
   p.kernel_name = nm;
diff --git a/compute-engine_amd/csrc/lce_plan.h b/compute-engine_amd/csrc/lce_plan.h
--- a/compute-engine_amd/csrc/lce_plan.h
+++ b/compute-engine_amd/csrc/lce_plan.h
@@ -56,6 +56,7 @@
   int stream_strip_pref = -1;
   int stream_interleave_pref = -1;
   int stream_occ_pref = 0;
+  int stream_tile_pref = 0;
   int ws_blocks_pref = 0, ws_images_pref = 0;
   bool cus_forced = false;
 };
@@ -113,6 +114,8 @@
   int st_occ = 1;
   int st_flat = 0;
   int st_nq = 0;
+  int st_tile_steps = 4;
+  int st_item_b = 0;
   int st_spb = 0, st_gx = 0, st_rows = 0, st_ring_bytes = 0, st_batch = 0;
   std::vector<uint32_t> st_tabs;
   uint32_t st_tab_lim = 0, st_tab_ctx = 0, st_tab_sgn = 0, st_tab_seg = 0;
@@ -199,6 +202,9 @@
 inline int stream_blocks_per_cu_max(const HostPlan& p) {
   return p.d.dst_type == LCE_HIP_BITPACKED && stream_chunks(p.d) == 1 ? 2 : 1;
 }
+inline bool stream_tile8_instance(const HostPlan& p, bool strips) {
+  return p.d.dst_type == LCE_HIP_F32 && stream_chunks(p.d) == 4 && !strips;
+}
 inline int stream_lds_bytes(const HostPlan& p) { return p.st_ring_bytes + stream_lds_extra(p); }
 
 }
diff --git a/compute-engine_amd/csrc/lce_plan_stream.cpp b/compute-engine_amd/csrc/lce_plan_stream.cpp
--- a/compute-engine_amd/csrc/lce_plan_stream.cpp
+++ b/compute-engine_amd/csrc/lce_plan_stream.cpp
@@ -23,8 +23,8 @@
   return kch == 1 || kch == 2 || kch == 4 || kch == 8;
 }
 
-static bool simulate_stream(const HostPlan& p, int rs, int spb, int pph_log, bool flat, int ow, int in_w, int* ring_rows,
-                            std::vector<uint32_t>* sched) {
+static bool simulate_stream(const HostPlan& p, int rs, int spb, int pph_log, bool flat, int ow, int in_w, int ts, int* ring_rows,
+                            std::vector<uint32_t>* sched, int* item_b) {
   const lce_hip_bconv2d_desc& d = p.d;
   const int kh = d.filter_height, sh = d.stride_height;
   const int srs = (rs - 1) * sh + kh, pbs = ceil_div(rs * ow, 32);
@@ -33,13 +33,15 @@
   const int pph = 1 << pph_log;
   const int64_t npx = (int64_t)rs * ow;
   const int64_t nblk = flat ? (spb * npx + 31) / 32 : (int64_t)spb * pbs;
-  const int64_t usteps = (nblk + pph - 1) / pph, ntile = (usteps + 3) / 4;
+  const int64_t usteps = (nblk + pph - 1) / pph;
+  const int64_t ntile = ts == 4 || usteps <= 4 ? (usteps + 3) / 4 : 1 + (usteps + 3) / 8;
+  auto tile_lo = [&](int64_t t) -> int64_t { return ts == 4 ? 4 * t : t == 0 ? 0 : 8 * t - 4; };
   const int64_t total = (int64_t)spb * srs * ipr;
   if (ntile < 1 || total >= (1ll << 31) || ntile > (1 << 20)) return false;
   std::vector<int64_t> need(ntile + 2), first(ntile);
   for (int64_t t = 0; t < ntile; ++t) {
     int64_t hi = 0, lo = INT64_MAX;
-    for (int64_t q = 4 * t * pph; q < std::min<int64_t>(nblk, 4 * (t + 1) * pph); ++q) {
+    for (int64_t q = tile_lo(t) * pph; q < std::min<int64_t>(nblk, tile_lo(t + 1) * pph); ++q) {
       if (flat) {
         const int64_t p0 = q * 32, p1 = std::min<int64_t>(q * 32 + 31, spb * npx - 1);
         lo = std::min(lo, (p0 / npx) * srs + (p0 % npx) / ow * sh);
@@ -56,16 +58,26 @@
   }
   need[ntile] = need[ntile + 1] = need[ntile - 1];
   for (int64_t t = 1; t < ntile; ++t) need[t] = std::max(need[t], need[t - 1]);
-  const int64_t cap = stream_ksplit(p) ? 768 : 512;
+  auto woven = [&](int64_t t) -> int64_t { return stream_ksplit(p) || (ts == 8 && t > 0) ? 512 : 256; };
   std::vector<int64_t> m(ntile + 2), s(ntile + 2);
-  m[ntile + 1] = m[ntile] = need[ntile];
-  for (int64_t t = ntile - 1; t >= 0; --t) m[t] = std::max(need[t], m[t + 1] - cap);
-  s[0] = m[0];
-  for (int64_t t = 0; t <= ntile; ++t) {
-    int64_t inc = 0;
-    while (s[t] + inc < m[t + 1]) inc += 256;
-    s[t + 1] = std::min(total, s[t] + inc);
-    if (s[t + 1] < m[t + 1] || inc > cap) return false;
+  auto produce = [&](int64_t extra) -> bool {
+    m[ntile + 1] = m[ntile] = need[ntile];
+    for (int64_t t = ntile - 1; t >= 0; --t) m[t] = std::max(need[t], m[t + 1] - (woven(t) + extra));
+    s[0] = m[0];
+    for (int64_t t = 0; t <= ntile; ++t) {
+      int64_t inc = 0;
+      while (s[t] + inc < m[t + 1]) inc += 256;
+      s[t + 1] = std::min(total, s[t] + inc);
+      if (s[t + 1] < m[t + 1] || inc > woven(t) + extra) return false;
+    }
+    return true;
+  };
+  if (!produce(256)) return false;
+  if (ts == 8) {
+    const int64_t rounds_b = (s[0] + 1023) / 1024;
+    if (!produce(0) || (s[0] + 1023) / 1024 > rounds_b) {
+      if (!produce(256)) return false;
+    }
   }
   int64_t rows = kh;
   for (int64_t t = 0; t < ntile; ++t)
@@ -73,6 +85,9 @@
   *ring_rows = (int)rows;
   sched->resize(ntile + 2);
   for (int64_t t = 0; t < ntile + 2; ++t) (*sched)[t] = (uint32_t)s[t];
+  *item_b = 0;
+  for (int64_t t = 0; t <= ntile; ++t)
+    if (s[t + 1] - s[t] > woven(t)) ++*item_b;
   return true;
 }
 
@@ -89,6 +104,9 @@
   const uint32_t row_bytes = stream_row_bytes(p);
   if ((int64_t)batch_chunk * p.out_h * p.out_w * row_bytes >= (1ll << 31))
     return "bconv2d: the streaming kernel binds the whole output of a launch to one buffer resource (< 2 GiB)";
+  if (p.stream_tile_pref == 8 && !stream_tile8_instance(p, p.stream_strip_pref > 0))
+    return "bconv2d: stream_tile_steps=8: tile steps of eight block steps exist for float output on the 256-channel filter bank "
+           "(193..256 input channels) and whole rows only";
   std::vector<int> widths;
   if (p.stream_strip_pref <= 0) widths.push_back(0);
   if (p.stream_strip_pref > 0 && stream_chunks(d) != 4)
@@ -98,12 +116,13 @@
       if (p.stream_strip_pref % 32 != 0 || p.out_w % p.stream_strip_pref != 0)
         return "bconv2d: stream_strip must be a multiple of 32 that divides the output width";
       widths.push_back(p.stream_strip_pref);
-    } else if (p.out_w % 32 == 0 && p.out_w > 64) {
+    } else if (p.out_w % 32 == 0 && p.out_w > 64 && p.stream_tile_pref != 8) {
       if (p.out_w % 64 == 0) widths.push_back(64);
       widths.push_back(32);
     }
   }
-  std::string why = pick.occ == 2 ? "bconv2d: stream_blocks_per_cu=2: two blocks' row rings do not fit a CU's LDS for this layer"
+  std::string why = p.stream_tile_pref == 8 ? "bconv2d: stream_tile_steps=8: the row ring of eight block steps per tile step does not fit LDS for this layer"
+                    : pick.occ == 2 ? "bconv2d: stream_blocks_per_cu=2: two blocks' row rings do not fit a CU's LDS for this layer"
                                            : "bconv2d: the streaming kernel's row ring does not fit LDS for this layer";
   for (int wso : widths)
     if (plan_stream_geometry(p, batch_chunk, pick, wso, &why)) return "";
@@ -162,9 +181,22 @@
     int rows = 0;
     std::vector<uint32_t> sched;
     const bool flat = !strips && rs == p.out_h && spb > 1 && (rs * p.out_w) % 32 != 0 && !p.stream_noflat && ksplit;
-    if (!simulate_stream(p, rs, (int)spb, pph_log, flat, ow_seg, in_w_seg, &rows, &sched)) continue;
-    const int64_t ring = ((int64_t)rows * pitch + 1023) / 1024 * 1024;
-    if ((ring + stream_lds_extra(p)) * occ > 160 * 1024) continue;
+    const int64_t seg_steps = (ceil_div(rs * ow_seg, 32) + pph - 1) / pph;
+    const bool try8 = p.stream_tile_pref == 8 || (p.stream_tile_pref == 0 && stream_tile8_instance(p, strips) && !flat && seg_steps >= 16);
+    int item_b = 0, tsteps = 0;
+    int64_t ring = 0;
+    for (int ts : {8, 4}) {
+      if (ts == 8 ? !try8 : p.stream_tile_pref == 8) continue;
+      if (!simulate_stream(p, rs, (int)spb, pph_log, flat, ow_seg, in_w_seg, ts, &rows, &sched, &item_b)) continue;
+      if (ts == 8 && p.stream_tile_pref == 0 && item_b > 0) continue;
+      ring = ((int64_t)rows * pitch + 1023) / 1024 * 1024;
+      if ((ring + stream_lds_extra(p)) * occ > 160 * 1024) continue;
+      tsteps = ts;
+      break;
+    }
+    if (!tsteps) continue;
+    p.st_tile_steps = tsteps;
+    p.st_item_b = item_b;
     p.st_occ = occ;
     const int pbs = ceil_div(rs * ow_seg, 32);
     if (strips && (rs * ow_seg) % 32 != 0) continue;
@@ -184,8 +216,9 @@
     p.wp = wp;
     if (p.dbg_level >= 2)
       fprintf(stderr,
-              "[lce plan] stream geometry: rows/segment %d, ring %d rows x %d B = %lld B (+%d), blocks %d x %d, segments/block %lld\n",
-              rs, rows, pitch, (long long)ring, stream_lds_extra(p), p.st_gx, ny, (long long)spb);
+              "[lce plan] stream geometry: rows/segment %d, ring %d rows x %d B = %lld B (+%d), blocks %d x %d, segments/block %lld, %d block steps "
+              "per tile step (%d with the out-of-line item)\n",
+              rs, rows, pitch, (long long)ring, stream_lds_extra(p), p.st_gx, ny, (long long)spb, tsteps, item_b);
     p.st_pitch = pitch;
     const size_t n_sched = (sched.size() + 3) / 4 * 4, n_lim = ((size_t)nq + 3) / 4 * 4;
     const size_t n_sgn = d.dst_type == LCE_HIP_BITPACKED ? 0 : (size_t)nq * 64;
@@ -257,6 +290,7 @@
   G.flat = p.st_flat;
   G.NPX = p.st_rs * p.out_w;
   G.NQ = p.st_nq;
+  G.TS = p.st_tile_steps;
   G.need0 = p.st_tabs.empty() ? 0u : p.st_tabs[0];
   G.in_bytes = (uint32_t)((int64_t)batch_chunk * d.in_height * d.in_width * p.cw * 4);
   G.w_bytes = (uint32_t)p.wq.size();
```

Result: no change. 2678000 billion, median of 6 (+0.2%).
